# matter-labs/era-zkevm_test_harness

Measured on AMD Instinct MI355X. Metric: base-layer circuits/sec (2^20 rows); full-block synth wall-time 1/8 GPU, higher is better.
Workload: dtype u64 (Goldilocks, p = 2^64 - 2^32 + 1)

## Files before the change

### era_zkevm_test_harness_amd/csrc/poseidon2.cuh

```cuda
#pragma once
#include "gl64.cuh"
#include "../../include/zkw_poseidon2_params.h"

namespace p2 {
using gl::u32;
using gl::u64;

static __constant__ u64 c_rc[P2_TOTAL_ROUNDS * P2_WIDTH] = P2_ROUND_CONSTANTS_INIT;
static __constant__ u32 c_shift[P2_WIDTH] = P2_INTERNAL_DIAG_SHIFTS_INIT;

__host__ __device__ __forceinline__ u64 rc_at(int i) {
#if defined(__HIP_DEVICE_COMPILE__)
    return c_rc[i];
#else
    return P2_ROUND_CONSTANTS[i];
#endif
}
__host__ __device__ __forceinline__ u32 shift_at(int i) {
#if defined(__HIP_DEVICE_COMPILE__)
    return c_shift[i];
#else
    return P2_INTERNAL_DIAG_SHIFTS[i];
#endif
}

struct Wide {
    u64 lo;
    u32 hi;
};
GL_HD Wide wide(u64 x) { Wide r; r.lo = x; r.hi = 0; return r; }
GL_HD Wide wadd(Wide a, Wide b) {
    Wide r;
    r.lo = a.lo + b.lo;
    r.hi = a.hi + b.hi + (r.lo < a.lo ? 1u : 0u);
    return r;
}
GL_HD Wide wshl(Wide a, u32 s) {
    Wide r;
    r.lo = a.lo << s;
    r.hi = (a.hi << s) | (u32)(a.lo >> (64 - s));
    return r;
}
GL_HD u64 wreduce(Wide a) {
    u64 t = ((u64)a.hi << 32) - a.hi;
    u64 r = a.lo + t;
    u64 c = r < t ? gl::EPS : 0;
    return r + c;
}

GL_HD void m4w(const u64 x[4], Wide t[4]) {
    Wide t0 = wadd(wide(x[0]), wide(x[1])), t1 = wadd(wide(x[2]), wide(x[3]));
    Wide t2 = wadd(wshl(wide(x[1]), 1), t1), t3 = wadd(wshl(wide(x[3]), 1), t0);
    Wide t4 = wadd(wshl(t1, 2), t3), t5 = wadd(wshl(t0, 2), t2);
    t[0] = wadd(t3, t5); t[1] = t5; t[2] = wadd(t2, t4); t[3] = t4;
}

#if defined(__HIP_DEVICE_COMPILE__)
__device__ __forceinline__ u64 mad_acc(u32 a, u32 k, u64 acc) {
    u64 r, dead;
    asm("v_mad_u64_u32 %0, %1, %2, %3, %4" : "=v"(r), "=s"(dead) : "v"(a), "s"(k), "v"(acc));
    return r;
}
__device__ __forceinline__ u64 mad_acc1(u32 a, u64 acc) {
    u64 r, dead;
    asm("v_mad_u64_u32 %0, %1, %2, 1, %3" : "=v"(r), "=s"(dead) : "v"(a), "v"(acc));
    return r;
}
__device__ __forceinline__ u64 mad_acc2(u32 a, u64 acc) {
    u64 r, dead;
    asm("v_mad_u64_u32 %0, %1, %2, 2, %3" : "=v"(r), "=s"(dead) : "v"(a), "v"(acc));
    return r;
}
__device__ __forceinline__ u64 wp_reduce(u64 L, u64 H) {
    const u32 l0 = (u32)L, l1 = (u32)(L >> 32), h0 = (u32)H, h1 = (u32)(H >> 32);
    u32 n1, k, f;
    u64 c, c2, dead, r;
    asm("v_add_co_u32_e64 %0, %1, %2, %3" : "=v"(n1), "=s"(c) : "v"(l1), "v"(h0));
    asm("v_addc_co_u32_e64 %0, %1, %2, 0, %3" : "=v"(k), "=s"(dead) : "v"(h1), "s"(c));
    const u64 x = ((u64)n1 << 32) | l0;
    asm("v_mad_u64_u32 %0, %1, %2, -1, %3" : "=v"(r), "=s"(c2) : "v"(k), "v"(x));
    asm("v_cndmask_b32_e64 %0, 0, 1, %1" : "=v"(f) : "s"(c2));
    asm("v_mad_u64_u32 %0, %1, %2, -1, %3" : "=v"(r), "=s"(dead) : "v"(f), "v"(r));
    return r;
}
__device__ __forceinline__ void m4_plane(u32 a0, u32 a1, u32 a2, u32 a3, u64 y[4]) {
    const u64 t0 = mad_acc1(a0, (u64)a1), t1 = mad_acc1(a2, (u64)a3);
    const u64 t2 = mad_acc2(a1, t1), t3 = mad_acc2(a3, t0);
    const u64 t4 = (t1 << 2) + t3, t5 = (t0 << 2) + t2;
    y[0] = t3 + t5; y[1] = t5; y[2] = t2 + t4; y[3] = t4;
}
#endif

GL_HD void external(u64 s[12]) {
#if defined(__HIP_DEVICE_COMPILE__) && !defined(P2_LINEAR_WIDE)
    u64 L[12], H[12];
#pragma unroll
    for (int b = 0; b < 3; b++) {
        m4_plane((u32)s[4 * b], (u32)s[4 * b + 1], (u32)s[4 * b + 2], (u32)s[4 * b + 3], L + 4 * b);
        m4_plane((u32)(s[4 * b] >> 32), (u32)(s[4 * b + 1] >> 32), (u32)(s[4 * b + 2] >> 32), (u32)(s[4 * b + 3] >> 32), H + 4 * b);
    }
#pragma unroll
    for (int i = 0; i < 4; i++) {
        const u64 cl = L[i] + L[4 + i] + L[8 + i], ch = H[i] + H[4 + i] + H[8 + i];
#pragma unroll
        for (int b = 0; b < 3; b++) s[4 * b + i] = wp_reduce(L[4 * b + i] + cl, H[4 * b + i] + ch);
    }
#else
    Wide t[12];
    m4w(s, t); m4w(s + 4, t + 4); m4w(s + 8, t + 8);
#pragma unroll
    for (int i = 0; i < 4; i++) {
        Wide col = wadd(wadd(t[i], t[4 + i]), t[8 + i]);
        s[i] = wreduce(wadd(t[i], col)); s[4 + i] = wreduce(wadd(t[4 + i], col)); s[8 + i] = wreduce(wadd(t[8 + i], col));
    }
#endif
}

GL_HD void internal(u64 s[12]) {
    constexpr u32 SH[12] = P2_INTERNAL_DIAG_SHIFTS_INIT;
#if defined(__HIP_DEVICE_COMPILE__) && !defined(P2_LINEAR_WIDE)
    u64 sl = (u64)(u32)s[0], sh = s[0] >> 32;
#pragma unroll
    for (int i = 1; i < 12; i++) { sl = mad_acc1((u32)s[i], sl); sh = mad_acc1((u32)(s[i] >> 32), sh); }
#pragma unroll
    for (int i = 0; i < 12; i++) {
        const u64 l = SH[i] ? mad_acc((u32)s[i], 1u << SH[i], sl) : mad_acc1((u32)s[i], sl);
        const u64 h = SH[i] ? mad_acc((u32)(s[i] >> 32), 1u << SH[i], sh) : mad_acc1((u32)(s[i] >> 32), sh);
        s[i] = wp_reduce(l, h);
    }
#else
    Wide sum = wide(s[0]);
#pragma unroll
    for (int i = 1; i < 12; i++) sum = wadd(sum, wide(s[i]));
#pragma unroll
    for (int i = 0; i < 12; i++) s[i] = wreduce(wadd(SH[i] ? wshl(wide(s[i]), SH[i]) : wide(s[i]), sum));
#endif
}

#ifndef P2_SBOX_GROUP
#define P2_SBOX_GROUP 3
#endif
template <bool LAT = false>
GL_HD void full_round(u64 s[12], int r) {
#pragma unroll
    for (int i = 0; i < 12; i++) {
        s[i] = LAT ? gl::pow7_lat(gl::add_canon(s[i], rc_at(12 * r + i))) : gl::pow7(gl::add_canon(s[i], rc_at(12 * r + i)));
#if defined(__HIP_DEVICE_COMPILE__)
        if (!LAT && (i + 1) % P2_SBOX_GROUP == 0) __builtin_amdgcn_sched_barrier(0);
#endif
    }
    external(s);
}

template <bool LAT = false>
GL_HD void partial_round(u64 s[12], int r) {
    s[0] = LAT ? gl::pow7_lat(gl::add_canon(s[0], rc_at(12 * r))) : gl::pow7(gl::add_canon(s[0], rc_at(12 * r)));
    internal(s);
}

template <bool LAT = false>
GL_HD void permute(u64 s[12]) {
    external(s);
    int r = 0;
    for (int k = 0; k < P2_HALF_FULL_ROUNDS; k++, r++) full_round<LAT>(s, r);
    for (int k = 0; k < P2_PARTIAL_ROUNDS; k++, r++) partial_round<LAT>(s, r);
    for (int k = 0; k < P2_HALF_FULL_ROUNDS; k++, r++) full_round<LAT>(s, r);
}
GL_HD void permute_lat(u64 s[12]) { permute<true>(s); }

#if defined(__HIPCC__)
template <int CTRL>
__device__ __forceinline__ u32 dpp32(u32 v) {
    return (u32)__builtin_amdgcn_update_dpp((int)0, (int)v, CTRL, 0xF, 0xF, false);
}
template <int CTRL>
__device__ __forceinline__ u64 dpp64(u64 v) {
    u32 lo = dpp32<CTRL>((u32)v), hi = dpp32<CTRL>((u32)(v >> 32));
    return ((u64)hi << 32) | lo;
}
constexpr int QP_ROT1 = 1 | (2 << 2) | (3 << 4) | (0 << 6);
constexpr int QP_ROT2 = 2 | (3 << 2) | (0 << 4) | (1 << 6);
constexpr int QP_ROT3 = 3 | (0 << 2) | (1 << 4) | (2 << 6);
constexpr int QP_SWAP1 = 1 | (0 << 2) | (3 << 4) | (2 << 6);
constexpr int QP_BCAST0 = 0;
constexpr int ROW_ROR4 = 0x124, ROW_ROR8 = 0x128, ROW_ROR12 = 0x12C;

template <int CTRL>
__device__ __forceinline__ Wide wdpp(Wide a) {
    Wide r;
    r.lo = dpp64<CTRL>(a.lo);
    r.hi = dpp32<CTRL>(a.hi);
    return r;
}
__device__ __forceinline__ u64 add_rc_sched(u64 x, u64 c) {
    u32 r0, r1, m;
    asm("v_add_co_u32 %0, vcc, %3, %5\n\t"
        "v_addc_co_u32 %1, vcc, %4, %6, vcc\n\t"
        "v_cndmask_b32 %2, 0, -1, vcc\n\t"
        "v_add_co_u32 %0, vcc, %0, %2\n\t"
        "v_addc_co_u32 %1, vcc, 0, %1, vcc"
        : "=&v"(r0), "=&v"(r1), "=&v"(m)
        : "v"((u32)x), "v"((u32)(x >> 32)), "v"((u32)c), "v"((u32)(c >> 32))
        : "vcc");
    return ((u64)r1 << 32) | r0;
}
#if defined(GL_CHAIN_MUL_COMPILER_FORM)
#define P2_ROW_MUL gl::mul_sched
#else
#define P2_ROW_MUL gl::mul_vcc
#endif
__device__ __forceinline__ u64 pow7_sched(u64 x) {
    const u64 x2 = P2_ROW_MUL(x, x), x3 = P2_ROW_MUL(x2, x), x4 = P2_ROW_MUL(x2, x2);
    return P2_ROW_MUL(x3, x4);
}

struct Coop {
    u64 rc_full[2 * P2_HALF_FULL_ROUNDS];
    u32 ka, kb, kd;
    u32 shift;
    u32 rsh, hi_mask;
    bool active;
    bool first;
    bool second;

    __device__ __forceinline__ void init(int g) {
        active = g < 12;
        first = g == 0;
        second = g == 1;
#pragma unroll
        for (int k = 0; k < 2 * P2_HALF_FULL_ROUNDS; k++) {
            int round = k < P2_HALF_FULL_ROUNDS ? k : k + P2_PARTIAL_ROUNDS;
            rc_full[k] = active ? c_rc[12 * round + g] : 0;
        }
        bool even = (g & 1) == 0;
        ka = even ? 5u : 6u;
        kb = even ? 7u : 1u;
        kd = even ? 3u : 4u;
        shift = active ? c_shift[g] : 0;
        rsh = (32u - shift) & 31u;
        hi_mask = shift ? 0xffffffffu : 0u;
    }

    __device__ __forceinline__ u64 external(u64 x) const {
        u64 a = x, b = dpp64<QP_ROT1>(x), c = dpp64<QP_ROT2>(x), d = dpp64<QP_ROT3>(x);
        u64 L = (a & gl::EPS) * ka + (b & gl::EPS) * kb + (c & gl::EPS) + (d & gl::EPS) * kd;
        u64 H = (a >> 32) * ka + (b >> 32) * kb + (c >> 32) + (d >> 32) * kd;
        u32 r0, r1, t0, t1, t2, u0, u1, u2, e0, e1, e2;
        asm volatile(
            "v_add_co_u32 %3, vcc, %11, %13\n\t"
            "v_addc_co_u32 %4, vcc, 0, %14, vcc\n\t"
            "s_nop 0\n\t"
            "v_add_co_u32_dpp %5, vcc, %12, %12 row_ror:8 row_mask:0xf bank_mask:0xf\n\t"
            "v_addc_co_u32_dpp %6, vcc, %3, %3, vcc row_ror:8 row_mask:0xf bank_mask:0xf\n\t"
            "v_addc_co_u32_dpp %7, vcc, %4, %4, vcc row_ror:8 row_mask:0xf bank_mask:0xf\n\t"
            "v_add_co_u32_dpp %5, vcc, %5, %5 row_ror:4 row_mask:0xf bank_mask:0xf\n\t"
            "v_addc_co_u32_dpp %6, vcc, %6, %6, vcc row_ror:4 row_mask:0xf bank_mask:0xf\n\t"
            "v_addc_co_u32_dpp %7, vcc, %7, %7, vcc row_ror:4 row_mask:0xf bank_mask:0xf\n\t"
            "v_add_co_u32 %0, vcc, %12, %5\n\t"
            "v_addc_co_u32 %1, vcc, %3, %6, vcc\n\t"
            "v_addc_co_u32 %2, vcc, %4, %7, vcc\n\t"
            "v_sub_co_u32 %8, vcc, 0, %2\n\t"
            "v_subbrev_co_u32 %9, vcc, 0, %2, vcc\n\t"
            "v_add_co_u32 %0, vcc, %0, %8\n\t"
            "v_addc_co_u32 %1, vcc, %1, %9, vcc\n\t"
            "v_cndmask_b32 %10, 0, -1, vcc\n\t"
            "v_add_co_u32 %0, vcc, %0, %10\n\t"
            "v_addc_co_u32 %1, vcc, 0, %1, vcc"
            : "=&v"(r0), "=&v"(r1), "=&v"(t0), "=&v"(t1), "=&v"(t2), "=&v"(u0), "=&v"(u1), "=&v"(u2), "=&v"(e0), "=&v"(e1), "=&v"(e2)
            : "v"((u32)(L >> 32)), "v"((u32)L), "v"((u32)H), "v"((u32)(H >> 32))
            : "vcc");
        const u64 y = ((u64)r1 << 32) | r0;
        return active ? y : 0;
    }

    __device__ __forceinline__ u64 internal(u64 x) const {
        const u32 x0 = (u32)x, x1 = (u32)(x >> 32);
        u32 s0, s1, s2;
        const u32 zero = 0;
        asm volatile(
            "s_nop 1\n\t"
            "v_add_co_u32_dpp %0, vcc, %3, %3 row_ror:8 row_mask:0xf bank_mask:0xf\n\t"
            "v_addc_co_u32_dpp %1, vcc, %4, %4, vcc row_ror:8 row_mask:0xf bank_mask:0xf\n\t"
            "v_addc_co_u32 %2, vcc, 0, %5, vcc\n\t"
            "v_add_co_u32_dpp %0, vcc, %0, %0 row_ror:4 row_mask:0xf bank_mask:0xf\n\t"
            "v_addc_co_u32_dpp %1, vcc, %1, %1, vcc row_ror:4 row_mask:0xf bank_mask:0xf\n\t"
            "v_addc_co_u32_dpp %2, vcc, %2, %2, vcc row_ror:4 row_mask:0xf bank_mask:0xf\n\t"
            "v_add_co_u32_dpp %0, vcc, %0, %0 quad_perm:[2,3,0,1] row_mask:0xf bank_mask:0xf\n\t"
            "v_addc_co_u32_dpp %1, vcc, %1, %1, vcc quad_perm:[2,3,0,1] row_mask:0xf bank_mask:0xf\n\t"
            "v_addc_co_u32_dpp %2, vcc, %2, %2, vcc quad_perm:[2,3,0,1] row_mask:0xf bank_mask:0xf\n\t"
            "v_add_co_u32_dpp %0, vcc, %0, %0 quad_perm:[1,0,3,2] row_mask:0xf bank_mask:0xf\n\t"
            "v_addc_co_u32_dpp %1, vcc, %1, %1, vcc quad_perm:[1,0,3,2] row_mask:0xf bank_mask:0xf\n\t"
            "v_addc_co_u32_dpp %2, vcc, %2, %2, vcc quad_perm:[1,0,3,2] row_mask:0xf bank_mask:0xf"
            : "=&v"(s0), "=&v"(s1), "=&v"(s2)
            : "v"(x0), "v"(x1), "v"(zero)
            : "vcc");
        const u64 mlo = x << shift;
        const u32 m2 = (x1 >> rsh) & hi_mask;
        u32 r0, r1;
        u32 t0, t1, t2, t3;
        asm volatile(
            "v_add_co_u32 %0, vcc, %6, %9\n\t"
            "v_addc_co_u32 %1, vcc, %7, %10, vcc\n\t"
            "v_addc_co_u32 %2, vcc, %8, %11, vcc\n\t"
            "v_sub_co_u32 %3, vcc, 0, %2\n\t"
            "v_subbrev_co_u32 %4, vcc, 0, %2, vcc\n\t"
            "v_add_co_u32 %0, vcc, %0, %3\n\t"
            "v_addc_co_u32 %1, vcc, %1, %4, vcc\n\t"
            "v_cndmask_b32 %5, 0, -1, vcc\n\t"
            "v_add_co_u32 %0, vcc, %0, %5\n\t"
            "v_addc_co_u32 %1, vcc, 0, %1, vcc"
            : "=&v"(r0), "=&v"(r1), "=&v"(t0), "=&v"(t1), "=&v"(t2), "=&v"(t3)
            : "v"((u32)mlo), "v"((u32)(mlo >> 32)), "v"(m2), "v"(s0), "v"(s1), "v"(s2)
            : "vcc");
        const u64 y = ((u64)r1 << 32) | r0;
        return active ? y : 0;
    }

    __device__ __forceinline__ u64 permute(u64 x) const {
        x = external(x);
#pragma unroll
        for (int k = 0; k < P2_HALF_FULL_ROUNDS; k++) x = external(pow7_sched(add_rc_sched(x, rc_full[k])));
        for (int k = 0; k < P2_PARTIAL_ROUNDS; k++) {
            u64 rc = c_rc[12 * (P2_HALF_FULL_ROUNDS + k)];
            u64 sx = pow7_pair(add_rc_sched(x, rc));
            x = internal(first ? sx : x);
        }
#pragma unroll
        for (int k = 0; k < P2_HALF_FULL_ROUNDS; k++)
            x = external(pow7_sched(add_rc_sched(x, rc_full[P2_HALF_FULL_ROUNDS + k])));
        return x;
    }

    __device__ __forceinline__ u64 pow7_pair(u64 t) const {
        const u64 t0 = dpp64<QP_BCAST0>(t);
        const u64 x2 = P2_ROW_MUL(t0, t0);
        const u64 b = second ? x2 : t0;
        const u64 y = P2_ROW_MUL(x2, b);
        return P2_ROW_MUL(y, dpp64<QP_SWAP1>(y));
    }
};

template <class Put>
__device__ __forceinline__ u64 coop_flattened(const Coop& co, u64 x, u32 g, Put&& put) {
    if (co.active) put(g, gl::canon(x));
    x = co.external(x);
#pragma unroll
    for (int k = 0; k < P2_HALF_FULL_ROUNDS; k++) {
        x = co.external(pow7_sched(add_rc_sched(x, co.rc_full[k])));
        if (co.active) put(12 * (k + 1) + g, gl::canon(x));
    }
    for (int k = 0; k < P2_PARTIAL_ROUNDS; k++) {
        const u64 rc = c_rc[12 * (P2_HALF_FULL_ROUNDS + k)];
        const u64 sx = co.pow7_pair(add_rc_sched(x, rc));
        if (co.first) put(12 * (P2_HALF_FULL_ROUNDS + 1) + k, gl::canon(sx));
        x = co.internal(co.first ? sx : x);
    }
#pragma unroll
    for (int k = 0; k < P2_HALF_FULL_ROUNDS; k++) {
        x = co.external(pow7_sched(add_rc_sched(x, co.rc_full[P2_HALF_FULL_ROUNDS + k])));
        if (co.active) put(12 * (P2_HALF_FULL_ROUNDS + 1) + P2_PARTIAL_ROUNDS + 12 * k + g, gl::canon(x));
    }
    return gl::canon(x);
}


__device__ __forceinline__ u64 q4_mul(u64 a, u64 b) {
#if defined(GL_CHAIN_MUL_COMPILER_FORM)
    return gl::mul_lat(a, b);
#else
    return gl::mul_vcc(a, b);
#endif
}
__device__ __forceinline__ u64 q4_pow7(u64 x) {
    const u64 x2 = q4_mul(x, x), x3 = q4_mul(x2, x), x4 = q4_mul(x2, x2);
    return q4_mul(x3, x4);
}
template <int CTRL>
__device__ __forceinline__ u32 qdpp32(u32 v) {
    return (u32)__builtin_amdgcn_update_dpp((int)0, (int)v, CTRL, 0xF, 0xF, true);
}
template <int CTRL>
__device__ __forceinline__ u64 qdpp64(u64 v) {
    return ((u64)qdpp32<CTRL>((u32)(v >> 32)) << 32) | qdpp32<CTRL>((u32)v);
}

struct Coop4 {
    u64 rc_full[2 * P2_HALF_FULL_ROUNDS][3];
    u32 ka, kb, kd;
    u32 pw[3];
    bool first;
    bool second;

    __device__ __forceinline__ void init(int j) {
        first = j == 0;
        second = j == 1;
#pragma unroll
        for (int k = 0; k < 2 * P2_HALF_FULL_ROUNDS; k++) {
            int round = k < P2_HALF_FULL_ROUNDS ? k : k + P2_PARTIAL_ROUNDS;
#pragma unroll
            for (int c = 0; c < 3; c++) rc_full[k][c] = c_rc[12 * round + 4 * c + j];
        }
        bool even = (j & 1) == 0;
        ka = even ? 5u : 6u;
        kb = even ? 7u : 1u;
        kd = even ? 3u : 4u;
#pragma unroll
        for (int c = 0; c < 3; c++) pw[c] = 1u << c_shift[4 * c + j];
    }

#if defined(__HIP_DEVICE_COMPILE__)
    static __device__ __forceinline__ u64 mad_v(u32 a, u32 k, u64 acc) {
        u64 r, dead;
        asm("v_mad_u64_u32 %0, %1, %2, %3, %4" : "=v"(r), "=s"(dead) : "v"(a), "v"(k), "v"(acc));
        return r;
    }
    template <bool SC = false>
    static __device__ __forceinline__ u64 add_rc(u64 x, u32 c0, u32 c1);
#endif

    __device__ __forceinline__ u64 m4_plane(u32 a) const {
        const u32 b = qdpp32<QP_ROT1>(a), c = qdpp32<QP_ROT2>(a), d = qdpp32<QP_ROT3>(a);
#if defined(__HIP_DEVICE_COMPILE__)
        return mad_v(d, kd, mad_v(b, kb, mad_v(a, ka, (u64)c)));
#else
        return (u64)a * ka + (u64)b * kb + c + (u64)d * kd;
#endif
    }

    __device__ __forceinline__ void external(u64 x[3]) const {
#if defined(__HIP_DEVICE_COMPILE__)
        u64 L[3], H[3];
#pragma unroll
        for (int c = 0; c < 3; c++) { L[c] = m4_plane((u32)x[c]); H[c] = m4_plane((u32)(x[c] >> 32)); }
        const u64 cl = L[0] + L[1] + L[2], ch = H[0] + H[1] + H[2];
#pragma unroll
        for (int c = 0; c < 3; c++) x[c] = wp_reduce(L[c] + cl, H[c] + ch);
#endif
    }

    __device__ __forceinline__ void internal(u64 x[3]) const {
#if defined(__HIP_DEVICE_COMPILE__)
        const u64 pl = mad_acc1((u32)x[0], mad_acc1((u32)x[1], (u64)(u32)x[2]));
        const u64 ph = mad_acc1((u32)(x[0] >> 32), mad_acc1((u32)(x[1] >> 32), x[2] >> 32));
        u32 l0, l1, h0, h1;
        asm volatile(
            "s_nop 1\n\t"
            "v_add_co_u32_dpp %0, vcc, %4, %4 quad_perm:[2,3,0,1] row_mask:0xf bank_mask:0xf\n\t"
            "v_addc_co_u32_dpp %1, vcc, %5, %5, vcc quad_perm:[2,3,0,1] row_mask:0xf bank_mask:0xf\n\t"
            "v_add_co_u32_dpp %2, vcc, %6, %6 quad_perm:[2,3,0,1] row_mask:0xf bank_mask:0xf\n\t"
            "v_addc_co_u32_dpp %3, vcc, %7, %7, vcc quad_perm:[2,3,0,1] row_mask:0xf bank_mask:0xf\n\t"
            "v_add_co_u32_dpp %0, vcc, %0, %0 quad_perm:[1,0,3,2] row_mask:0xf bank_mask:0xf\n\t"
            "v_addc_co_u32_dpp %1, vcc, %1, %1, vcc quad_perm:[1,0,3,2] row_mask:0xf bank_mask:0xf\n\t"
            "v_add_co_u32_dpp %2, vcc, %2, %2 quad_perm:[1,0,3,2] row_mask:0xf bank_mask:0xf\n\t"
            "v_addc_co_u32_dpp %3, vcc, %3, %3, vcc quad_perm:[1,0,3,2] row_mask:0xf bank_mask:0xf"
            : "=&v"(l0), "=&v"(l1), "=&v"(h0), "=&v"(h1)
            : "v"((u32)pl), "v"((u32)(pl >> 32)), "v"((u32)ph), "v"((u32)(ph >> 32))
            : "vcc");
        const u64 sl = ((u64)l1 << 32) | l0, sh = ((u64)h1 << 32) | h0;
#pragma unroll
        for (int c = 0; c < 3; c++) x[c] = wp_reduce(mad_v((u32)x[c], pw[c], sl), mad_v((u32)(x[c] >> 32), pw[c], sh));
// ... 132 lines not shown
```

### era_zkevm_test_harness_amd/csrc/ram_circuit_kernels.cuh

```cuda
#pragma once
#include "../../include/zkw_ram_circuit_spec.h"
#include "../../include/zkw_decommit_sorter_circuit_spec.h"
#include "../../include/zkw_events_sorter_circuit_spec.h"
#include "ram_kernels.cuh"
#include "public_input_kernels.cuh"
#include "closed_form_kernels.cuh"

namespace zkw {

struct SynthJob {
    const zkw_ram_instance* inst;
    const zkw_mem_query* sorted_q;
    const zkw_mem_query* unsorted_q;
    const u64* unsorted_caps;
    const u64* sorted_caps;
    const u64* u_mark;
    const u64* s_mark;
    const u64* challenges;
    const u64* lhs_z;
    const u64* rhs_z;
    u64 n_block;
    u64* trace;
    u32* hist;
    u32* nd_tiles;
    const u64* public_input;
    const zkw_ram_instance* first_inst;
    u32 tail_clean;
};

constexpr int ROW_SLOTS[RC_NUM_ROW_TYPES] = RC_ROW_NUM_SLOTS_INIT;
constexpr int ROW_LOOKUPS[RC_NUM_ROW_TYPES] = RC_ROW_NUM_LOOKUPS_INIT;
static_assert(ROW_SLOTS[RC_ROW_PU] == 133 && ROW_SLOTS[RC_ROW_PS] == 130, "Poseidon2 rows: 130 gate variables (+3 spare in PU)");
static_assert(ROW_LOOKUPS[RC_ROW_PU] == 12 && ROW_LOOKUPS[RC_ROW_PS] == 12 && ROW_LOOKUPS[RC_ROW_A] == 12 &&
              ROW_LOOKUPS[RC_ROW_B] == 12 && ROW_LOOKUPS[RC_ROW_C] == 8 && ROW_LOOKUPS[RC_ROW_D] == 0,
              "lookup cells per cycle (56) are hard-wired in the fill kernels");
constexpr int LOOKUPS_PER_CYCLE = 56;

__device__ __forceinline__ u64 inv_or_zero(u64 x) { return gl::canon(x) ? gl::inv(x) : 0; }

struct RegsIn {
    const u64* uh;
    const u64* sh;
    u32 len;
};
__device__ __forceinline__ RegsIn regs_in(const zkw_ram_instance* in) {
    RegsIn r;
    const bool start = in->start_flag != 0;
    r.uh = start ? in->unsorted_queue_initial_state.head : in->hidden_fsm_input.current_unsorted_queue_state.head;
    r.sh = start ? in->sorted_queue_initial_state.head : in->hidden_fsm_input.current_sorted_queue_state.head;
    r.len = start ? in->unsorted_queue_initial_state.length : in->hidden_fsm_input.current_unsorted_queue_state.length;
    return r;
}

#define TR(col, row) trace[(size_t)(col) * n_rows + (row)]

__device__ __forceinline__ void zero_gap_row(u64* trace, size_t n_rows, size_t row) {
    for (int col = 0; col < RC_G + RC_L; col++) TR(col, row) = 0;
}
__device__ __forceinline__ void zero_gap_row_n(u64* trace, size_t n_rows, size_t row, int n_cols) {
    for (int col = 0; col < n_cols; col++) TR(col, row) = 0;
}

__device__ __forceinline__ void hist_bytes(u32* sh_hist, u32 x) {
    atomicAdd(&sh_hist[x & 0xFF], 1u);
    atomicAdd(&sh_hist[(x >> 8) & 0xFF], 1u);
    atomicAdd(&sh_hist[(x >> 16) & 0xFF], 1u);
    atomicAdd(&sh_hist[x >> 24], 1u);
}
__device__ __forceinline__ void put_bytes(u64* trace, size_t n_rows, size_t row, int col0, u32 x) {
    TR(col0, row) = x & 0xFF;
    TR(col0 + 1, row) = (x >> 8) & 0xFF;
    TR(col0 + 2, row) = (x >> 16) & 0xFF;
    TR(col0 + 3, row) = x >> 24;
}
__device__ __forceinline__ void hist_flush(u32* sh_hist, u32* g_hist) {
    __syncthreads();
    for (int t = threadIdx.x; t < 256; t += blockDim.x)
        if (sh_hist[t]) atomicAdd(&g_hist[t], sh_hist[t]);
}

__device__ __forceinline__ void fill_flattened_poseidon(u64* trace, size_t n_rows, size_t row, u64 s[12]) {
    int pos = 0;
#pragma unroll
    for (int k = 0; k < 12; k++) TR(pos++, row) = gl::canon(s[k]);
    p2::external(s);
    int r = 0;
    for (int k = 0; k < P2_HALF_FULL_ROUNDS; k++, r++) {
        p2::full_round(s, r);
#pragma unroll
        for (int j = 0; j < 12; j++) TR(pos + j, row) = gl::canon(s[j]);
        pos += 12;
    }
    for (int k = 0; k < P2_PARTIAL_ROUNDS; k++, r++) {
        s[0] = gl::pow7(gl::add_canon(s[0], p2::rc_at(12 * r)));
        TR(pos++, row) = gl::canon(s[0]);
        p2::internal(s);
    }
    for (int k = 0; k < P2_HALF_FULL_ROUNDS; k++, r++) {
        p2::full_round(s, r);
#pragma unroll
        for (int j = 0; j < 12; j++) TR(pos + j, row) = gl::canon(s[j]);
        pos += 12;
    }
}

template <int SIDE>
static __device__ __forceinline__ void k_ram_fill_poseidon(const VB& vb, const SynthJob* __restrict__ jobs, u32 capacity,
                                                          size_t n_rows) {
    __shared__ u32 sh_hist[256];
    for (int t = threadIdx.x; t < 256; t += blockDim.x) sh_hist[t] = 0;
    __syncthreads();
    const SynthJob job = jobs[vb.y];
    const u32 i = vb.x * blockDim.x + threadIdx.x;
    if (i < capacity) {
        u64* trace = job.trace;
        const zkw_ram_instance* in = job.inst;
        const size_t first = in->first_item, m = in->num_items;
        const bool can_pop = i < m;
        const size_t row = (size_t)(SIDE == 0 ? RC_ROW_PU : RC_ROW_PS) * RC_REGION_STRIDE(capacity) + i;
        const zkw_mem_query* qs = SIDE == 0 ? job.unsorted_q : job.sorted_q;
        const u64* caps = SIDE == 0 ? job.unsorted_caps : job.sorted_caps;
        u64 s[12];
        if (can_pop) {
            encode_raw_query(load_raw_query(qs + first + i), s);
        } else {
#pragma unroll
            for (int k = 0; k < 8; k++) s[k] = 0;
        }
        const RegsIn ri = regs_in(in);
        const u64* prev_cap = i == 0 ? (SIDE == 0 ? ri.uh : ri.sh) + 8 : caps + 4 * (first + (i - 1 < m ? i - 1 : m - 1));
#pragma unroll
        for (int k = 0; k < 4; k++) s[8 + k] = prev_cap[k];
        fill_flattened_poseidon(trace, n_rows, row, s);
        zkw_mem_query q;
        memset(&q, 0, sizeof q);
        if (can_pop) q = job.sorted_q[first + i];
        if (SIDE == 0) {
            TR(RC_PU_idx, row) = q.index; TR(RC_PU_v0, row) = q.value[0]; TR(RC_PU_v1, row) = q.value[1];
            put_bytes(trace, n_rows, row, RC_PU_idx_b0, q.index);
            put_bytes(trace, n_rows, row, RC_PU_v0_b0, q.value[0]);
            put_bytes(trace, n_rows, row, RC_PU_v1_b0, q.value[1]);
            hist_bytes(sh_hist, q.index); hist_bytes(sh_hist, q.value[0]); hist_bytes(sh_hist, q.value[1]);
        } else {
            if (!job.tail_clean) for (int c = 130; c < RC_G; c++) TR(c, row) = 0;
            put_bytes(trace, n_rows, row, RC_PS_ts_b0, q.timestamp);
            put_bytes(trace, n_rows, row, RC_PS_page_b0, q.page);
            put_bytes(trace, n_rows, row, RC_PS_v4_b0, q.value[4]);
            hist_bytes(sh_hist, q.timestamp); hist_bytes(sh_hist, q.page); hist_bytes(sh_hist, q.value[4]);
        }
        if (!job.tail_clean) for (int c = RC_G + 12; c < RC_G + RC_L; c++) TR(c, row) = 0;
    } else if (i < RC_REGION_STRIDE(capacity)) {
        if (!job.tail_clean) zero_gap_row(job.trace, n_rows, (size_t)(SIDE == 0 ? RC_ROW_PU : RC_ROW_PS) * RC_REGION_STRIDE(capacity) + i);
    }
    hist_flush(sh_hist, job.hist);
}

struct CycleCtx {
    bool can_pop;
    zkw_mem_query q, pq;
    u64 eu[8], es[8];
    u64 p_val[5];
    u32 p_ptr;
};

__device__ __forceinline__ void load_query(const zkw_mem_query* src, zkw_mem_query& dst) {
    const uint4* s = reinterpret_cast<const uint4*>(src);
    uint4* d = reinterpret_cast<uint4*>(&dst);
    d[0] = s[0]; d[1] = s[1]; d[2] = s[2];
}

__device__ __forceinline__ void cycle_ctx(const SynthJob& job, u32 i, CycleCtx& c, bool want_eu) {
    const zkw_ram_instance* in = job.inst;
    const size_t first = in->first_item, m = in->num_items;
    c.can_pop = i < m;
    memset(&c.q, 0, sizeof c.q);
    memset(&c.pq, 0, sizeof c.pq);
#pragma unroll
    for (int k = 0; k < 8; k++) { c.eu[k] = 0; c.es[k] = 0; }
    if (c.can_pop) {
        load_query(job.sorted_q + first + i, c.q);
        encode_mem_query(c.q, c.es);
        if (want_eu) encode_raw_query(load_raw_query(job.unsorted_q + first + i), c.eu);
    }
    if (i == 0) {
        const zkw_ram_fsm& f = in->hidden_fsm_input;
        c.pq.timestamp = f.previous_sorting_key[0]; c.pq.index = f.previous_sorting_key[1]; c.pq.page = f.previous_sorting_key[2];
        for (int k = 0; k < 8; k++) c.pq.value[k] = f.previous_value[k];
        c.pq.value_is_pointer = f.previous_is_ptr ? 1 : 0;
    } else if (i - 1 < m) {
        load_query(job.sorted_q + first + i - 1, c.pq);
    }
    u64 pe[8];
    encode_mem_query(c.pq, pe);
#pragma unroll
    for (int k = 0; k < 5; k++) c.p_val[k] = pe[3 + k];
    c.p_ptr = c.pq.value_is_pointer ? 1 : 0;
}

__device__ __forceinline__ u64 acc_before(const u64* z, size_t first, size_t m, u32 i, u64 fsm_in) {
    return i == 0 ? fsm_in : z[first + (i - 1 < m ? i - 1 : m - 1)];
}

static __device__ __forceinline__ void k_ram_fill_A(const VB& vb, const SynthJob* __restrict__ jobs, u32 capacity, size_t n_rows) {
    __shared__ u32 sh_hist[256];
    sh_hist[threadIdx.x] = 0;
    __syncthreads();
    const SynthJob job = jobs[vb.y];
    const u32 i = vb.x * blockDim.x + threadIdx.x;
    const u64* lhs_z_all = job.lhs_z;
    const u64* rhs_z_all = job.rhs_z;
    const size_t n_total = job.n_block;
    if (i < capacity) {
        u64* trace = job.trace;
        const zkw_ram_instance* in = job.inst;
        const size_t first = in->first_item, m = in->num_items, row = (size_t)RC_ROW_A * RC_REGION_STRIDE(capacity) + i;
        CycleCtx c;
        cycle_ctx(job, i, c, true);
        const u64 rw = c.q.rw_flag ? 1 : 0, ptr = c.q.value_is_pointer ? 1 : 0;
#pragma unroll
        for (int k = 0; k < 8; k++) { TR(RC_A_eu0 + k, row) = c.eu[k]; TR(RC_A_ts + k, row) = c.es[k]; }
        for (int r = 0; r < 2; r++) {
            const u64* ch = job.challenges + 9 * r;
            u64 lc = ch[8], rc = ch[8];
#pragma unroll
            for (int k = 0; k < 8; k++) {
                lc = gl::add(lc, gl::mul(c.eu[k], ch[k]));
                rc = gl::add(rc, gl::mul(c.es[k], ch[k]));
            }
            const u64 pl = acc_before(lhs_z_all + (size_t)r * n_total, first, m, i, in->hidden_fsm_input.lhs_accumulator[r]);
            const u64 pr = acc_before(rhs_z_all + (size_t)r * n_total, first, m, i, in->hidden_fsm_input.rhs_accumulator[r]);
            const u64 nl = gl::canon(gl::mul(pl, lc)), nr = gl::canon(gl::mul(pr, rc));
            const int o = r * (RC_A_lc1 - RC_A_lc0);
#pragma unroll
            for (int k = 1; k < 9; k++) TR(RC_A_G_c0_1 + (k - 1) + r * (RC_A_G_c1_1 - RC_A_G_c0_1), row) = ch[k];
            TR(RC_A_lc0 + o, row) = gl::canon(lc); TR(RC_A_P_lhs0 + o, row) = pl; TR(RC_A_nl0 + o, row) = nl;
            TR(RC_A_lhs0 + o, row) = c.can_pop ? nl : pl;
            TR(RC_A_rc0 + o, row) = gl::canon(rc); TR(RC_A_P_rhs0 + o, row) = pr; TR(RC_A_nr0 + o, row) = nr;
            TR(RC_A_rhs0 + o, row) = c.can_pop ? nr : pr;
        }
        TR(RC_A_rw, row) = rw; TR(RC_A_ptr, row) = ptr; TR(RC_A_idx, row) = c.q.index;
        TR(RC_A_v2, row) = c.q.value[2]; TR(RC_A_v3, row) = c.q.value[3]; TR(RC_A_v0, row) = c.q.value[0];
        TR(RC_A_v5_b3c, row) = c.q.value[5] >> 24; TR(RC_A_can_pop, row) = c.can_pop ? 1 : 0;
        put_bytes(trace, n_rows, row, RC_A_v2_b0, c.q.value[2]);
        put_bytes(trace, n_rows, row, RC_A_v3_b0, c.q.value[3]);
        put_bytes(trace, n_rows, row, RC_A_v5_b0, c.q.value[5]);
        hist_bytes(sh_hist, c.q.value[2]); hist_bytes(sh_hist, c.q.value[3]); hist_bytes(sh_hist, c.q.value[5]);
        constexpr int NA = ROW_SLOTS[RC_ROW_A];
        if (!job.tail_clean) {
            for (int col = NA; col < RC_G; col++) TR(col, row) = 0;
            for (int col = RC_G + 12; col < RC_G + RC_L; col++) TR(col, row) = 0;
        }
    } else if (i < RC_REGION_STRIDE(capacity)) {
        if (!job.tail_clean) zero_gap_row(job.trace, n_rows, (size_t)RC_ROW_A * RC_REGION_STRIDE(capacity) + i);
    }
    hist_flush(sh_hist, job.hist);
}

static __device__ __forceinline__ void k_ram_fill_B(const VB& vb, const SynthJob* __restrict__ jobs, u32 capacity, size_t n_rows) {
    __shared__ u32 sh_hist[256];
    sh_hist[threadIdx.x] = 0;
    __syncthreads();
    const SynthJob job = jobs[vb.y];
    const u32 i = vb.x * blockDim.x + threadIdx.x;
    if (i < capacity) {
        u64* trace = job.trace;
        const size_t row = (size_t)RC_ROW_B * RC_REGION_STRIDE(capacity) + i;
        CycleCtx c;
        cycle_ctx(job, i, c, false);
        put_bytes(trace, n_rows, row, RC_B_v6_b0, c.q.value[6]);
        put_bytes(trace, n_rows, row, RC_B_v7_b0, c.q.value[7]);
        TR(RC_B_es4, row) = c.es[4]; TR(RC_B_v1, row) = c.q.value[1]; TR(RC_B_v5_b3c, row) = c.q.value[5] >> 24;
        TR(RC_B_es5, row) = c.es[5]; TR(RC_B_v2, row) = c.q.value[2];
        TR(RC_B_es6, row) = c.es[6]; TR(RC_B_v3, row) = c.q.value[3];
        const u32 d0 = c.q.timestamp - c.pq.timestamp;
        TR(RC_B_d0, row) = d0; put_bytes(trace, n_rows, row, RC_B_d0_b0, d0);
        TR(RC_B_bw0, row) = c.q.timestamp < c.pq.timestamp ? 1 : 0;
        TR(RC_B_ts, row) = c.q.timestamp; TR(RC_B_P_ts, row) = c.pq.timestamp;
        hist_bytes(sh_hist, c.q.value[6]); hist_bytes(sh_hist, c.q.value[7]); hist_bytes(sh_hist, d0);
        constexpr int NB = ROW_SLOTS[RC_ROW_B];
        if (!job.tail_clean) {
            for (int col = NB; col < RC_G; col++) TR(col, row) = 0;
            for (int col = RC_G + 12; col < RC_G + RC_L; col++) TR(col, row) = 0;
        }
    } else if (i < RC_REGION_STRIDE(capacity)) {
        if (!job.tail_clean) zero_gap_row(job.trace, n_rows, (size_t)RC_ROW_B * RC_REGION_STRIDE(capacity) + i);
    }
    hist_flush(sh_hist, job.hist);
}

__device__ __forceinline__ bool nd_flag(bool can_pop, const zkw_mem_query& q) {
    return can_pop && q.timestamp == 0 && q.page == RC_HEAP_PAGE && q.rw_flag && !q.value_is_pointer;
}

static __device__ __forceinline__ void k_ram_nd_tiles(const VB& vb, const SynthJob* __restrict__ jobs, u32 capacity) {
    __shared__ u32 sh[4];
    const SynthJob job = jobs[vb.y];
    const u32 i = vb.x * blockDim.x + threadIdx.x;
    const zkw_ram_instance* in = job.inst;
    bool f = false;
    if (i < capacity && i < in->num_items) {
        zkw_mem_query q;
        load_query(job.sorted_q + in->first_item + i, q);
        f = nd_flag(true, q);
    }
    u32 cnt = __popcll(__ballot(f));
    if ((threadIdx.x & 63) == 0) sh[threadIdx.x >> 6] = cnt;
    __syncthreads();
    if (threadIdx.x == 0) job.nd_tiles[vb.x] = sh[0] + sh[1] + sh[2] + sh[3];
}
static __device__ __forceinline__ void k_ram_nd_scan(const VB& vb, const SynthJob* __restrict__ jobs, int n_jobs, u32 n_tiles) {
    u32* t = jobs[vb.x].nd_tiles;
    const int lane = threadIdx.x;
    u32 acc = 0;
    for (u32 base = 0; base < n_tiles; base += 64) {
        const u32 k = base + lane;
        const u32 v = k < n_tiles ? t[k] : 0;
        u32 incl = v;
        for (int off = 1; off < 64; off <<= 1) {
            const u32 up = __shfl_up(incl, off);
            if (lane >= off) incl += up;
        }
        if (k < n_tiles) t[k] = acc + incl - v;
        acc += __shfl(incl, 63);
    }
}

static __device__ __forceinline__ void k_ram_fill_C(const VB& vb, const SynthJob* __restrict__ jobs, u32 capacity, size_t n_rows) {
    __shared__ u32 sh_hist[256];
    __shared__ u32 sh_wave[4];
    sh_hist[threadIdx.x] = 0;
    __syncthreads();
    const SynthJob job = jobs[vb.y];
    const u32 i = vb.x * blockDim.x + threadIdx.x;
    const bool live = i < capacity;
    CycleCtx c;
    c.can_pop = false;
    bool nd = false;
    if (live) {
        cycle_ctx(job, i, c, false);
        nd = nd_flag(c.can_pop, c.q);
    }
    const unsigned long long bal = __ballot(nd);
    const int lane = threadIdx.x & 63, wave = threadIdx.x >> 6;
    if (lane == 0) sh_wave[wave] = __popcll(bal);
    __syncthreads();
    u32 before = __popcll(bal & ((1ull << lane) - 1));
    for (int w = 0; w < wave; w++) before += sh_wave[w];
    if (live) {
        u64* trace = job.trace;
        const zkw_ram_instance* in = job.inst;
        const size_t row = (size_t)RC_ROW_C * RC_REGION_STRIDE(capacity) + i;
        const u64 rw = c.q.rw_flag ? 1 : 0, ptr = c.q.value_is_pointer ? 1 : 0;
        const u64 bw0 = c.q.timestamp < c.pq.timestamp ? 1 : 0;
        const u64 t1 = (u64)c.pq.index + bw0, bw1 = (u64)c.q.index < t1 ? 1 : 0;
        const u32 d1 = (u32)((u64)c.q.index - t1);
        const u64 t2 = (u64)c.pq.page + bw1, bw2 = (u64)c.q.page < t2 ? 1 : 0;
        const u32 d2 = (u32)((u64)c.q.page - t2);
        TR(RC_C_d1, row) = d1; put_bytes(trace, n_rows, row, RC_C_d1_b0, d1);
        TR(RC_C_d2, row) = d2; put_bytes(trace, n_rows, row, RC_C_d2_b0, d2);
        hist_bytes(sh_hist, d1); hist_bytes(sh_hist, d2);
        TR(RC_C_bw1, row) = bw1; TR(RC_C_bw2, row) = bw2; TR(RC_C_bw0, row) = bw0;
        TR(RC_C_idx, row) = c.q.index; TR(RC_C_P_idx, row) = c.pq.index;
        TR(RC_C_page, row) = c.q.page; TR(RC_C_P_page, row) = c.pq.page;
        TR(RC_C_can_pop, row) = c.can_pop ? 1 : 0;
        u64 x[14];
        x[0] = gl::canon(gl::sub(c.q.index, c.pq.index));
        x[1] = gl::canon(gl::sub(c.q.page, c.pq.page));
        const u64 val[5] = {c.es[3], c.es[4], c.es[5], c.es[6], c.es[7]};
#pragma unroll
        for (int k = 0; k < 5; k++) { x[2 + k] = gl::canon(gl::sub(val[k], c.p_val[k])); x[7 + k] = val[k]; }
        x[12] = c.q.timestamp;
        x[13] = gl::canon(gl::sub(c.q.page, RC_HEAP_PAGE));
        u64 pre[14], acc = 1;
#pragma unroll
        for (int k = 0; k < 14; k++) { pre[k] = acc; acc = gl::mul(acc, x[k] ? x[k] : 1); }
        u64 inv = gl::inv(acc), w[14];
#pragma unroll
        for (int k = 13; k >= 0; k--) {
            w[k] = x[k] ? gl::canon(gl::mul(inv, pre[k])) : 0;
            inv = gl::mul(inv, x[k] ? x[k] : 1);
        }
        const u64 z_idx = x[0] == 0, z_page = x[1] == 0, same = z_idx & z_page;
        TR(RC_C_w_idx, row) = w[0]; TR(RC_C_z_idx, row) = z_idx;
        TR(RC_C_w_page, row) = w[1]; TR(RC_C_z_page, row) = z_page; TR(RC_C_same, row) = same;
        const int C_VAL[5] = {RC_C_es3, RC_C_es4, RC_C_es5, RC_C_es6, RC_C_v4};
        const int C_PVAL[5] = {RC_C_P_es3, RC_C_P_es4, RC_C_P_es5, RC_C_P_es6, RC_C_P_v4};
        const int C_WEQ[5] = {RC_C_w_eq0, RC_C_w_eq1, RC_C_w_eq2, RC_C_w_eq3, RC_C_w_eq4};
        const int C_ZEQ[5] = {RC_C_z_eq0, RC_C_z_eq1, RC_C_z_eq2, RC_C_z_eq3, RC_C_z_eq4};
        const int C_WZ[5] = {RC_C_w_z0, RC_C_w_z1, RC_C_w_z2, RC_C_w_z3, RC_C_w_z4};
        const int C_ZZ[5] = {RC_C_z_z0, RC_C_z_z1, RC_C_z_z2, RC_C_z_z3, RC_C_z_z4};
        u64 zeq[5], zz[5];
#pragma unroll
        for (int k = 0; k < 5; k++) {
            zeq[k] = x[2 + k] == 0; zz[k] = x[7 + k] == 0;
            TR(C_VAL[k], row) = val[k]; TR(C_PVAL[k], row) = c.p_val[k];
            TR(C_WEQ[k], row) = w[2 + k]; TR(C_ZEQ[k], row) = zeq[k];
            TR(C_WZ[k], row) = w[7 + k]; TR(C_ZZ[k], row) = zz[k];
        }
        const u64 peq = ptr == c.p_ptr, eq_a = zeq[0] & zeq[1] & zeq[2], value_equal = eq_a & zeq[3] & zeq[4] & peq;
        const u64 zz_a = zz[0] & zz[1] & zz[2], all_zero = zz_a & zz[3] & zz[4] & (1 - ptr);
        TR(RC_C_ptr, row) = ptr; TR(RC_C_P_ptr, row) = c.p_ptr; TR(RC_C_peq, row) = peq;
        TR(RC_C_eq_a, row) = eq_a; TR(RC_C_value_equal, row) = value_equal;
        TR(RC_C_zz_a, row) = zz_a; TR(RC_C_all_zero, row) = all_zero; TR(RC_C_rw, row) = rw;
        TR(RC_C_ts, row) = c.q.timestamp; TR(RC_C_w_ts, row) = w[12]; TR(RC_C_z_ts, row) = x[12] == 0;
        TR(RC_C_w_heap, row) = w[13]; TR(RC_C_z_heap, row) = x[13] == 0; TR(RC_C_nd, row) = nd ? 1 : 0;
        const u64 p_cnt = (u64)in->hidden_fsm_input.num_nondeterministic_writes + job.nd_tiles[vb.x] + before;
        TR(RC_C_P_cnt, row) = p_cnt; TR(RC_C_cnt, row) = p_cnt + (nd ? 1 : 0);
        constexpr int NC = ROW_SLOTS[RC_ROW_C];
        if (!job.tail_clean) {
            for (int col = NC; col < RC_G; col++) TR(col, row) = 0;
            for (int col = RC_G + 8; col < RC_G + RC_L; col++) TR(col, row) = 0;
        }
    } else if (i < RC_REGION_STRIDE(capacity)) {
        if (!job.tail_clean) zero_gap_row(job.trace, n_rows, (size_t)RC_ROW_C * RC_REGION_STRIDE(capacity) + i);
    }
    if (vb.x == 0 && threadIdx.x == 0)
        for (int l = 5; l < 8; l++) { hist_bytes(sh_hist, job.inst->hidden_fsm_input.previous_value[l]); hist_bytes(sh_hist, job.inst->hidden_fsm_output.previous_value[l]); }
    hist_flush(sh_hist, job.hist);
}

__device__ __forceinline__ void ram_boundary_block(const SynthJob& job, u32 capacity, size_t n_rows);
constexpr int RC_D_TILES = 4;
static __device__ __forceinline__ void k_ram_fill_D(const VB& vb, const SynthJob* __restrict__ jobs, u32 n_jobs, u32 n_tiles, u32 capacity, size_t n_rows) {
    if (vb.x < n_jobs) {
        __builtin_amdgcn_s_setprio(3);
        ram_boundary_block(jobs[vb.x], capacity, n_rows);
        return;
    }
    const SynthJob& job = jobs[(vb.x - n_jobs) / n_tiles];
    const u32 i0 = ((vb.x - n_jobs) % n_tiles) * (RC_D_TILES * 256) + threadIdx.x;
    const size_t rs = RC_REGION_STRIDE(capacity);
    u64* trace = job.trace;
    const zkw_ram_instance* in = job.inst;
    const size_t m = in->num_items;
    const RegsIn ri = regs_in(in);
    u64 len[RC_D_TILES], pre[RC_D_TILES], w[RC_D_TILES];
    u64 acc = 1;
#pragma unroll
    for (int k = 0; k < RC_D_TILES; k++) {
        const u32 i = i0 + 256 * k;
        len[k] = (u64)ri.len - (i < m ? i : m);
        pre[k] = acc;
        acc = gl::mul(acc, len[k] ? len[k] : 1);
    }
    acc = gl::inv(acc);
#pragma unroll
    for (int k = RC_D_TILES - 1; k >= 0; k--) {
        w[k] = len[k] ? gl::canon(gl::mul(acc, pre[k])) : 0;
        acc = gl::mul(acc, len[k] ? len[k] : 1);
    }
#pragma unroll
    for (int k = 0; k < RC_D_TILES; k++) {
        const u32 i = i0 + 256 * k;
        if (i >= capacity) {
            if (i < rs && !job.tail_clean) zero_gap_row(job.trace, n_rows, (size_t)RC_ROW_D * rs + i);
            continue;
        }
        const size_t row = (size_t)RC_ROW_D * rs + i;
        const size_t rPU = (size_t)RC_ROW_PU * rs + i, rPS = (size_t)RC_ROW_PS * rs + i;
        const bool can_pop = i < m;
        const u64 p_len = len[k];
        const u64 w_len = w[k], z_len = p_len == 0;
        TR(RC_D_P_len_u, row) = p_len; TR(RC_D_w_lu, row) = w_len; TR(RC_D_z_lu, row) = z_len;
        TR(RC_D_P_len_s, row) = p_len; TR(RC_D_w_ls, row) = w_len; TR(RC_D_z_ls, row) = z_len;
        TR(RC_D_can_pop, row) = can_pop ? 1 : 0;
        TR(RC_D_len_u, row) = p_len - (can_pop ? 1 : 0); TR(RC_D_len_s, row) = p_len - (can_pop ? 1 : 0);
        const size_t p = i - 1 < m ? i - 1 : m - 1, rPUp = (size_t)RC_ROW_PU * rs + p, rPSp = (size_t)RC_ROW_PS * rs + p;
#pragma unroll
        for (int e = 0; e < 12; e++) {
            const u64 uo = TR(RC_PU_uo0 + e, rPU);
            const u64 so = TR(RC_PS_so0 + e, rPS);
            const u64 a = i == 0 ? ri.uh[e] : TR(RC_PU_uo0 + e, rPUp), b = i == 0 ? ri.sh[e] : TR(RC_PS_so0 + e, rPSp);
            const int o = 3 * e;
            TR(RC_D_uo0 + o, row) = uo; TR(RC_D_P_uh0 + o, row) = a; TR(RC_D_uh0 + o, row) = can_pop ? uo : a;
            TR(RC_D_so0 + o, row) = so; TR(RC_D_P_sh0 + o, row) = b; TR(RC_D_sh0 + o, row) = can_pop ? so : b;
        }
        constexpr int ND = ROW_SLOTS[RC_ROW_D];
        if (!job.tail_clean) for (int col = ND; col < RC_G + RC_L; col++) TR(col, row) = 0;
    }
}

constexpr int TAIL_CHUNKS = 8;
constexpr int RC_BOUNDARY_ROWS = RC_NUM_ROW_TYPES - RC_ROWS_PER_CYCLE;
constexpr int RC_CF_LOOKUP_CELLS = 24;
static_assert(RC_BOUNDARY_ROWS % 2 == 0, "the tail's 16-byte stores start below the boundary rows");
static __device__ __forceinline__ void k_ram_fill_tail(const VB& vb, const SynthJob* __restrict__ jobs, u32 capacity, size_t n_rows) {
    constexpr u32 PER_JOB = (RC_G + RC_L + 1) * TAIL_CHUNKS;
    const u32 bid = vb.x % PER_JOB;
    const SynthJob& job = jobs[vb.x / PER_JOB];
    u64* trace = job.trace;
    const int col = bid / TAIL_CHUNKS, ch = bid % TAIL_CHUNKS;
    if (col < RC_G + RC_L) {
        if (job.tail_clean) return;
        const size_t bnd = (size_t)RC_BOUNDARY_ROW(capacity) + RC_BOUNDARY_ROWS;
        const size_t n_pairs = (n_rows - bnd) / 2;
        const size_t per = (n_pairs + TAIL_CHUNKS - 1) / TAIL_CHUNKS, lo = ch * per, hi = lo + per < n_pairs ? lo + per : n_pairs;
        ulonglong2* c2 = reinterpret_cast<ulonglong2*>(trace + (size_t)col * n_rows + bnd);
        const ulonglong2 z = make_ulonglong2(0, 0);
        for (size_t k = lo + threadIdx.x; k < hi; k += 256) c2[k] = z;
        return;
    }
    u64* m = trace + (size_t)RC_MULT_COL * n_rows;
    const size_t per = (n_rows + TAIL_CHUNKS - 1) / TAIL_CHUNKS, lo = ch * per, hi = lo + per < n_rows ? lo + per : n_rows;
    for (size_t r = lo + threadIdx.x; r < (job.tail_clean && hi > 256 ? (lo < 256 ? 256 : lo) : hi); r += 256) {
        u64 v = 0;
        if (r < 256) {
            v = job.hist[r];
            if (r == 0) v += (u64)RC_L * n_rows - (u64)LOOKUPS_PER_CYCLE * capacity - RC_CF_LOOKUP_CELLS;
        }
        m[r] = v;
    }
}

static __constant__ rc_link c_links[RC_NUM_LINKS] = RC_LINKS_INIT;
static __constant__ uint8_t c_is_poseidon[RC_NUM_ROW_TYPES] = RC_ROW_IS_POSEIDON_INIT;
ZKW_CF_TABLES(RC, rc)

__device__ __forceinline__ void ram_fill_register_rows(const SynthJob& job, u32 capacity, size_t n_rows) {
    const u64* lhs_z_all = job.lhs_z;
    const u64* rhs_z_all = job.rhs_z;
    const size_t n_total = job.n_block;
    u64* trace = job.trace;
    const zkw_ram_instance* in = job.inst;
    const zkw_ram_fsm& fi = in->hidden_fsm_input;
    const size_t first = in->first_item, m = in->num_items;
    const size_t bin = (size_t)RC_BOUNDARY_ROW(capacity) + RC_ROWOFF_BND_IN, bout = bin - RC_ROWOFF_BND_IN + RC_ROWOFF_BND_OUT;
    const RegsIn ri = regs_in(in);
    for (int k = 0; k < 12; k++) { TR(RC_BND_IN_uh0 + k, bin) = ri.uh[k]; TR(RC_BND_IN_sh0 + k, bin) = ri.sh[k]; }
    TR(RC_BND_IN_len_u, bin) = ri.len; TR(RC_BND_IN_len_s, bin) = ri.len;
    for (int r = 0; r < 2; r++) { TR(RC_BND_IN_lhs0 + r, bin) = fi.lhs_accumulator[r]; TR(RC_BND_IN_rhs0 + r, bin) = fi.rhs_accumulator[r]; }
    zkw_mem_query pq;
    memset(&pq, 0, sizeof pq);
    for (int k = 0; k < 8; k++) pq.value[k] = fi.previous_value[k];
    u64 pe[8];
    encode_mem_query(pq, pe);
    TR(RC_BND_IN_ts, bin) = fi.previous_sorting_key[0]; TR(RC_BND_IN_idx, bin) = fi.previous_sorting_key[1];
    TR(RC_BND_IN_page, bin) = fi.previous_sorting_key[2];
    TR(RC_BND_IN_es3, bin) = pe[3]; TR(RC_BND_IN_es4, bin) = pe[4]; TR(RC_BND_IN_es5, bin) = pe[5];
    TR(RC_BND_IN_es6, bin) = pe[6]; TR(RC_BND_IN_v4, bin) = pe[7];
    TR(RC_BND_IN_ptr, bin) = fi.previous_is_ptr ? 1 : 0; TR(RC_BND_IN_cnt, bin) = fi.num_nondeterministic_writes;
    for (int r = 0; r < 2; r++)
        for (int k = 1; k < 9; k++) TR(RC_BND_IN_G_c0_1 + 8 * r + (k - 1), bin) = job.challenges[9 * r + k];
    const size_t last = first + m - 1;
    const bool padded = m < capacity;
    const u64 len_out = (u64)ri.len - m;
    for (int k = 0; k < 12; k++) {
        TR(RC_BND_OUT_uh0 + k, bout) = job.u_mark[k];
        TR(RC_BND_OUT_sh0 + k, bout) = job.s_mark[k];
        TR(RC_BND_OUT_tail_u0 + k, bout) = in->unsorted_queue_initial_state.tail[k];
        TR(RC_BND_OUT_tail_s0 + k, bout) = in->sorted_queue_initial_state.tail[k];
    }
    TR(RC_BND_OUT_len_u, bout) = len_out; TR(RC_BND_OUT_len_s, bout) = len_out;
    for (int r = 0; r < 2; r++) {
        TR(RC_BND_OUT_lhs0 + r, bout) = lhs_z_all[(size_t)r * n_total + last];
        TR(RC_BND_OUT_rhs0 + r, bout) = rhs_z_all[(size_t)r * n_total + last];
    }
    zkw_mem_query lq;
    memset(&lq, 0, sizeof lq);
    if (!padded) lq = job.sorted_q[last];
    u64 le[8];
    encode_mem_query(lq, le);
    TR(RC_BND_OUT_ts, bout) = lq.timestamp; TR(RC_BND_OUT_idx, bout) = lq.index; TR(RC_BND_OUT_page, bout) = lq.page;
    TR(RC_BND_OUT_es3, bout) = le[3]; TR(RC_BND_OUT_es4, bout) = le[4]; TR(RC_BND_OUT_es5, bout) = le[5];
    TR(RC_BND_OUT_es6, bout) = le[6]; TR(RC_BND_OUT_v4, bout) = le[7];
    TR(RC_BND_OUT_ptr, bout) = lq.value_is_pointer ? 1 : 0;
    TR(RC_BND_OUT_cnt, bout) = TR(RC_C_cnt, (size_t)RC_ROW_C * RC_REGION_STRIDE(capacity) + capacity - 1);
    TR(RC_BND_OUT_completion, bout) = in->completion_flag ? 1 : 0;
    TR(RC_BND_OUT_w_end, bout) = inv_or_zero(len_out); TR(RC_BND_OUT_z_end, bout) = len_out == 0;
}

__device__ __forceinline__ void ram_value_row(u64* trace, size_t n_rows, size_t row, int v0, int b0, int e3) {
    zkw_mem_query q;
    memset(&q, 0, sizeof q);
    for (int k = 0; k < 8; k++) q.value[k] = (u32)TR(v0 + k, row);
    for (int l = 5; l < 8; l++)
        for (int k = 0; k < 4; k++) {
            const u64 b = (q.value[l] >> (8 * k)) & 0xFF;
            TR(b0 + 4 * (l - 5) + k, row) = b;
        }
    if (e3 < 0) return;
    u64 e[8];
    encode_mem_query(q, e);
    for (int k = 0; k < 4; k++) TR(e3 + k, row) = e[3 + k];
}

__device__ __forceinline__ void ram_boundary_block(const SynthJob& job, u32 capacity, size_t n_rows) {
    {
        u64* trace = job.trace;
        const size_t bnd = (size_t)RC_BOUNDARY_ROW(capacity);
        for (int k = threadIdx.x; k < (RC_G + RC_L) * RC_BOUNDARY_ROWS; k += CF_THREADS) TR(k / RC_BOUNDARY_ROWS, bnd + k % RC_BOUNDARY_ROWS) = 0;
    }
    __syncthreads();
    __shared__ u64 sh_oi[RAM_INPUT_ENC_LEN], sh_fi[RAM_FSM_ENC_LEN], sh_fo[RAM_FSM_ENC_LEN], sh_flags[2];
    if (threadIdx.x == 0) ram_fill_register_rows(job, capacity, n_rows);
    if (threadIdx.x == 64) {
        int m = put_queue12(job.first_inst->unsorted_queue_initial_state, sh_oi);
        m += put_queue12(job.first_inst->sorted_queue_initial_state, sh_oi + m);
        sh_oi[m] = job.first_inst->non_deterministic_bootloader_memory_snapshot_length;
    }
    if (threadIdx.x == 128) ram_encode_fsm(job.inst->hidden_fsm_input, sh_fi);
    if (threadIdx.x == 192) {
        ram_encode_fsm(job.inst->hidden_fsm_output, sh_fo);
        sh_flags[0] = job.inst->start_flag ? 1 : 0;
        sh_flags[1] = job.inst->completion_flag ? 1 : 0;
    }
    __syncthreads();
    const CfSpec S = ZKW_CF_SPEC(RC, rc, c_is_poseidon);
    const CfSources src = {sh_oi, sh_fi, sh_fo, sh_flags, nullptr};
    u64* trace = job.trace;
    cf_fill_block(S, trace, n_rows, (size_t)RC_BOUNDARY_ROW(capacity), src, [&](int rt, size_t row) {
        if (threadIdx.x != 0) return;
        if (rt == RC_ROW_VIN) ram_value_row(trace, n_rows, row, RC_VIN_VIN_v0, RC_VIN_VIN_v5_b0, RC_VIN_VIN_e3);
        if (rt == RC_ROW_VOUT) ram_value_row(trace, n_rows, row, RC_VOUT_VOUT_v0, RC_VOUT_VOUT_v5_b0, -1);
    });
}

static __constant__ rc_term c_terms[RC_NUM_TERMS] = RC_TERMS_INIT;
static __constant__ rc_constraint c_cons[RC_NUM_CONSTRAINTS] = RC_CONSTRAINTS_INIT;
static __constant__ uint16_t c_row_first[RC_NUM_ROW_TYPES + 1] = RC_ROW_FIRST_CONSTRAINT_INIT;
static __constant__ rc_term c_ds_terms[DS_NUM_TERMS] = DS_TERMS_INIT;
static __constant__ rc_constraint c_ds_cons[DS_NUM_CONSTRAINTS] = DS_CONSTRAINTS_INIT;
static __constant__ uint16_t c_ds_row_first[DS_NUM_ROW_TYPES + 1] = DS_ROW_FIRST_CONSTRAINT_INIT;
static __constant__ uint8_t c_ds_is_poseidon[DS_NUM_ROW_TYPES] = DS_ROW_IS_POSEIDON_INIT;
static __constant__ rc_link c_ds_links[DS_NUM_LINKS] = DS_LINKS_INIT;

struct SpecRam {
    static constexpr int G = RC_G, L = RC_L, ROWS_PER_CYCLE = RC_ROWS_PER_CYCLE, NUM_ROW_TYPES = RC_NUM_ROW_TYPES, NUM_LINKS = RC_NUM_LINKS;
    static constexpr int OFF_BIN = RC_ROWOFF_BND_IN, OFF_BOUT = RC_ROWOFF_BND_OUT;
    __device__ static const rc_term* terms() { return c_terms; }
    __device__ static const rc_constraint* cons() { return c_cons; }
    __device__ static const uint16_t* row_first() { return c_row_first; }
    __device__ static const uint8_t* is_poseidon() { return c_is_poseidon; }
    __device__ static const rc_link* links() { return c_links; }
};
ZKW_CF_TABLES(DS, ds)
struct SpecDecommitSorter {
    static constexpr int G = DS_G, L = DS_L, ROWS_PER_CYCLE = DS_ROWS_PER_CYCLE, NUM_ROW_TYPES = DS_NUM_ROW_TYPES, NUM_LINKS = DS_NUM_LINKS;
    static constexpr int OFF_BIN = DS_ROWOFF_BND_IN, OFF_BOUT = DS_ROWOFF_BND_OUT;
    __device__ static const rc_term* terms() { return c_ds_terms; }
    __device__ static const rc_constraint* cons() { return c_ds_cons; }
    __device__ static const uint16_t* row_first() { return c_ds_row_first; }
    __device__ static const uint8_t* is_poseidon() { return c_ds_is_poseidon; }
    __device__ static const rc_link* links() { return c_ds_links; }
    ZKW_CF_SPEC_MEMBERS(DS, ds)
};
static __constant__ rc_term c_es_terms[ES_NUM_TERMS] = ES_TERMS_INIT;
static __constant__ rc_constraint c_es_cons[ES_NUM_CONSTRAINTS] = ES_CONSTRAINTS_INIT;
static __constant__ uint16_t c_es_row_first[ES_NUM_ROW_TYPES + 1] = ES_ROW_FIRST_CONSTRAINT_INIT;
static __constant__ uint8_t c_es_is_poseidon[ES_NUM_ROW_TYPES] = ES_ROW_IS_POSEIDON_INIT;
static __constant__ rc_link c_es_links[ES_NUM_LINKS] = ES_LINKS_INIT;
ZKW_CF_TABLES(ES, es)
struct SpecEventsSorter {
    static constexpr int G = ES_G, L = ES_L, ROWS_PER_CYCLE = ES_ROWS_PER_CYCLE, NUM_ROW_TYPES = ES_NUM_ROW_TYPES, NUM_LINKS = ES_NUM_LINKS;
    static constexpr int OFF_BIN = ES_ROWOFF_BND_IN, OFF_BOUT = ES_ROWOFF_BND_OUT;
    __device__ static const rc_term* terms() { return c_es_terms; }
    __device__ static const rc_constraint* cons() { return c_es_cons; }
    __device__ static const uint16_t* row_first() { return c_es_row_first; }
    __device__ static const uint8_t* is_poseidon() { return c_es_is_poseidon; }
    __device__ static const rc_link* links() { return c_es_links; }
    ZKW_CF_SPEC_MEMBERS(ES, es)
};

struct CheckResult {
    unsigned long long violations;
    unsigned long long first_bad;
};

__device__ __forceinline__ void flag_bad(CheckResult* res, u64 kind, u64 idx, u64 row) {
    atomicAdd(&res->violations, 1ull);
    atomicMin(&res->first_bad, (kind << 56) | (idx << 32) | row);
}

constexpr int CHK_ROWS = 64;

template <class S>
__device__ __forceinline__ size_t spec_row(int rt, u32 capacity, u32 i) {
    const size_t rs = RC_REGION_STRIDE(capacity);
    return rt < S::ROWS_PER_CYCLE ? (size_t)rt * rs + i : (size_t)S::ROWS_PER_CYCLE * rs + (rt - S::ROWS_PER_CYCLE);
}

template <class S>
static __global__ __launch_bounds__(64) void k_check_rows(const u64* __restrict__ trace, u32 capacity, size_t n_rows, CheckResult* res) {
    extern __shared__ __attribute__((aligned(16))) u64 tile[];
    constexpr int CHK_COLS = S::G + S::L;
    const int rt = blockIdx.y;
    const bool per_cycle = rt < S::ROWS_PER_CYCLE;
    const u32 n_in_region = per_cycle ? capacity : 1;
    const u32 i = blockIdx.x * CHK_ROWS + threadIdx.x;
    if (blockIdx.x * CHK_ROWS >= n_in_region) return;
    const bool live = i < n_in_region;
    const size_t row = spec_row<S>(rt, capacity, per_cycle ? i : 0);
    for (int c = 0; c < CHK_COLS; c++) {
        u64 v = live ? TR(c, row) : 0;
        tile[c * CHK_ROWS + threadIdx.x] = v;
        if (live && (v >= gl::P || (c >= S::G && v > 255))) flag_bad(res, 3, c, row);
    }
    __syncthreads();
    if (!live) return;
#define CELLV(c) tile[(c) * CHK_ROWS + threadIdx.x]
    for (int k = S::row_first()[rt]; k < S::row_first()[rt + 1]; k++) {
        const rc_constraint cn = S::cons()[k];
        u64 acc = 0;
        for (int t = 0; t < cn.n_terms; t++) {
            const rc_term* tm = &S::terms()[cn.first_term + t];
            u64 v = tm->coef;
            for (int f = 0; f < tm->nf; f++) v = gl::mul(v, CELLV(tm->f[f]));
            acc = gl::add(acc, v);
        }
        if (gl::canon(acc) != 0) flag_bad(res, 1, k, row);
    }
    if (S::is_poseidon()[rt]) {
        u64 s[12];
#pragma unroll
        for (int k = 0; k < 12; k++) s[k] = CELLV(k);
        int pos = 12, r = 0;
        bool ok = true;
        p2::external(s);
        for (int k = 0; k < P2_HALF_FULL_ROUNDS; k++, r++) {
            p2::full_round(s, r);
#pragma unroll
            for (int j = 0; j < 12; j++) ok &= gl::canon(s[j]) == CELLV(pos + j);
            pos += 12;
        }
        for (int k = 0; k < P2_PARTIAL_ROUNDS; k++, r++) {
            s[0] = gl::pow7(gl::add_canon(s[0], p2::rc_at(12 * r)));
            ok &= gl::canon(s[0]) == CELLV(pos);
            pos++;
            p2::internal(s);
        }
        for (int k = 0; k < P2_HALF_FULL_ROUNDS; k++, r++) {
            p2::full_round(s, r);
#pragma unroll
            for (int j = 0; j < 12; j++) ok &= gl::canon(s[j]) == CELLV(pos + j);
            pos += 12;
        }
        if (!ok) flag_bad(res, 2, 0, row);
    }
#undef CELLV
}

template <class S>
static __global__ __launch_bounds__(256) void k_check_links(const u64* __restrict__ trace, u32 capacity, size_t n_rows, CheckResult* res) {
    const u32 i = blockIdx.x * blockDim.x + threadIdx.x;
    if (i >= capacity) return;
    const size_t rs = RC_REGION_STRIDE(capacity), bnd = (size_t)S::ROWS_PER_CYCLE * rs;
    for (int l = 0; l < S::NUM_LINKS; l++) {
        const rc_link k = S::links()[l];
        if (k.kind == 3) {
            if (i == capacity - 1 && TR(k.col_a, bnd + S::OFF_BOUT) != TR(k.col_b, (size_t)k.row_b * rs + i))
                flag_bad(res, 4, l, bnd + S::OFF_BOUT);
            continue;
        }
        if (k.kind == 4) {
            if (i == 0 && TR(k.col_a, spec_row<S>(k.row_a, capacity, 0)) != TR(k.col_b, bnd + S::OFF_BOUT))
                flag_bad(res, 4, l, spec_row<S>(k.row_a, capacity, 0));
            continue;
        }
        if (k.kind == 5) {
            if (i == 0 && TR(k.col_a, spec_row<S>(k.row_a, capacity, 0)) != TR(k.col_b, spec_row<S>(k.row_b, capacity, 0)))
                flag_bad(res, 4, l, spec_row<S>(k.row_a, capacity, 0));
            continue;
        }
        const size_t ra = (size_t)k.row_a * rs + i;
        const u64 a = TR(k.col_a, ra);
        u64 b;
        if (k.kind == 0) b = TR(k.col_b, (size_t)k.row_b * rs + i);
        else if (k.kind == 1) b = i ? TR(k.col_b, (size_t)k.row_b * rs + i - 1) : TR(k.bin_col, bnd + S::OFF_BIN);
        else b = TR(k.col_b, bnd + S::OFF_BIN);
        if (a != b) flag_bad(res, 4, l, ra);
    }
}

template <class S>
static __global__ __launch_bounds__(256) void k_check_lookups(const u64* __restrict__ trace, u32 capacity, size_t n_rows,
                                                       u32* __restrict__ hist, CheckResult* res) {
    __shared__ u32 sh_hist[256];
    sh_hist[threadIdx.x] = 0;
    __syncthreads();
    const size_t rs = RC_REGION_STRIDE(capacity), pad0 = (size_t)S::ROWS_PER_CYCLE * rs + (S::NUM_ROW_TYPES - S::ROWS_PER_CYCLE);
    const size_t stride = (size_t)gridDim.x * blockDim.x;
    for (size_t r = (size_t)blockIdx.x * blockDim.x + threadIdx.x; r < n_rows; r += stride) {
        for (int c = S::G; c < S::G + S::L; c++) {
            const u64 v = TR(c, r);
            if (v > 255) flag_bad(res, 3, c, r); else atomicAdd(&sh_hist[v], 1u);
        }
        if (r >= pad0 || (r < (size_t)S::ROWS_PER_CYCLE * rs && r % rs >= capacity))
            for (int c = 0; c < S::G; c++)
                if (TR(c, r) != 0) { flag_bad(res, 6, c, r); break; }
    }
    __syncthreads();
    if (sh_hist[threadIdx.x]) atomicAdd(&hist[threadIdx.x], sh_hist[threadIdx.x]);
}
static __global__ void k_check_mult(const u64* __restrict__ trace, size_t n_rows, int mult_col, const u32* __restrict__ hist, CheckResult* res) {
    const size_t stride = (size_t)gridDim.x * blockDim.x;
    for (size_t r = (size_t)blockIdx.x * blockDim.x + threadIdx.x; r < n_rows; r += stride) {
        const u64 want = r < 256 ? hist[r] : 0;
        if (TR(mult_col, r) != want) flag_bad(res, 5, 0, r);
    }
}

#undef TR
}
```

### era_zkevm_test_harness_amd/csrc/zkw_api.hip

```cpp
#include "zkw_ctx.h"
#include "circuit_check_host.h"
#include "closed_forms_host.h"
#include "callstack_kernels.cuh"
#include "vm_kernels.cuh"
#include "radix_sort.cuh"

static thread_local std::string g_last_error;

#undef fail
int zkw_fail(int code, const char* fmt, ...) {
    char buf[512];
    va_list ap;
    va_start(ap, fmt);
    vsnprintf(buf, sizeof buf, fmt, ap);
    va_end(ap);
    g_last_error = buf;
    return code;
}

#define fail zkw_fail

struct AllocCache {
    static constexpr size_t SMALL_MAX = size_t(256) << 20;
    static constexpr int MAX_DEV = 16;
// ... 1156 lines not shown
    for (size_t b = 0; b < n_blocks; b++) {
        const size_t lo = w->offsets[b], n = w->offsets[b + 1] - lo;
        const size_t last_inst = w->inst_offsets[b + 1] - 1;
        fs[b] = FsJob{w->unsorted_marks + 12 * last_inst, w->sorted_marks + 12 * last_inst, (u32)n, (u32)n,
                      w->challenges + 18 * b};
    }
    ZKW_TRY(dev_fs(ctx, fs, 12, 9));
    w->z_valid = false;
    for (size_t b0 = 0; b0 < n_blocks;) {
        size_t b1 = b0 + 1;
        while (b1 < n_blocks && w->offsets[b1 + 1] - w->offsets[b0] <= w->zcap) b1++;
        ZKW_TRY(ram_gp_blocks(ctx, w, b0, b1, w->zbuf_l, w->zbuf_r));
        const size_t base = w->offsets[b0];
        std::vector<RamBlock> blocks(b1 - b0);
        size_t max_inst = 0;
        for (size_t b = b0; b < b1; b++) {
            const size_t lo = w->offsets[b], n = w->offsets[b + 1] - lo;
            const size_t n_inst = w->inst_offsets[b + 1] - w->inst_offsets[b];
            if (n_inst > max_inst) max_inst = n_inst;
            blocks[b - b0] = RamBlock{w->unsorted_q,
                                      w->perm + lo,
                                      w->unsorted_marks + 12 * w->inst_offsets[b],
                                      w->sorted_marks + 12 * w->inst_offsets[b],
                                      w->zbuf_l + 2 * (lo - base),
                                      w->zbuf_r + 2 * (lo - base),
                                      w->instances + w->inst_offsets[b],
                                      w->nondet_counts + w->inst_offsets[b],
                                      n,
                                      w->capacity,
                                      n_nondet ? n_nondet[b] : 0u};
        }
        RamBlock* d_blocks = nullptr;
        ZKW_TRY(ctx->upload("ram_blocks", blocks, &d_blocks));
        const unsigned gx = (unsigned)(max_inst < 64 ? max_inst : 64), gy = (unsigned)(b1 - b0);
        { Prof _p(ctx, "k_ram_count_nondet"); ZKW_LAUNCH_2D(ctx, k_ram_count_nondet, gx, gy, 256, d_blocks); }
        ZKW_TRY(launch_check("k_ram_count_nondet"));
        { Prof _p(ctx, "k_ram_instances"); ZKW_LAUNCH_2D(ctx, k_ram_instances, blocks_for(max_inst, 64), gy, 64, d_blocks); }
        ZKW_TRY(launch_check("k_ram_instances"));
        b0 = b1;
    }
    const size_t ni = w->n_instances;
    { Prof _p(ctx, "k_ram_commitments"); ZKW_LAUNCH(ctx, k_ram_commitments, blocks_for(4 * ni, 64), 64, w->instances, ni, w->compact_forms); }
    ZKW_TRY(launch_check("k_ram_commitments"));
    { Prof _p(ctx, "k_commit_encodings"); ZKW_LAUNCH(ctx, k_commit_encodings, blocks_for(ni, 64), 64, w->compact_forms, ni, (u32)COMPACT_FORM_LEN, w->public_inputs); }
    return launch_check("k_commit_encodings");
}

extern "C" int zkw_ram_build_instances_batch(zkw_ctx* ctx, const zkw_mem_query* q, const uint64_t* block_offsets,
                                             size_t n_blocks, uint32_t capacity, const uint32_t* n_nondet,
                                             zkw_ram_witness** out) {
    if (!ctx || !q || !block_offsets || !out || n_blocks == 0 || capacity == 0)
        return fail(ZKW_ERR_INVALID, "zkw_ram_build_instances_batch: bad argument");
    HIP_TRY(hipSetDevice(ctx->device));
    const uint64_t base = block_offsets[0];
    std::vector<uint64_t> offs(n_blocks + 1), ioffs(n_blocks + 1, 0);
    for (size_t b = 0; b <= n_blocks; b++) offs[b] = block_offsets[b] - base;
    for (size_t b = 0; b < n_blocks; b++) {
        if (block_offsets[b + 1] <= block_offsets[b])
            return fail(ZKW_ERR_INVALID, "block %zu is empty: the VM must have made memory requests "
                                         "(W/ram_permutation.rs:43-46)", b);
        ioffs[b + 1] = ioffs[b] + (offs[b + 1] - offs[b] + capacity - 1) / capacity;
    }
    const size_t total = offs[n_blocks];
    if (total >= (1ull << 32)) return fail(ZKW_ERR_INVALID, "more than 2^32-1 queries in one batch");
    zkw_ram_witness* w = *out;
    if (w && (w->ctx != ctx || w->offsets != offs || w->capacity != capacity)) {
        zkw_ram_witness_free(w);
        w = nullptr;
        *out = nullptr;
    }
    if (!w) {
        w = new zkw_ram_witness();
        w->ctx = ctx;
        w->offsets = offs;
        w->inst_offsets = ioffs;
        w->capacity = capacity;
        w->total = total;
        w->n_instances = ioffs[n_blocks];
        int rc = ram_alloc(w, n_blocks);
        if (rc != ZKW_OK) {
            w->release();
            delete w;
            return rc;
        }
    }
    const zkw_mem_query* d_q = nullptr;
    int rc = ctx->in("ram_q", q + base, total, &d_q);
    if (rc == ZKW_OK) rc = ram_run(ctx, w, d_q, n_nondet);
    if (rc == ZKW_OK) rc = ctx->sync_if_host();
    if (rc != ZKW_OK) {
        if (!*out) {
            w->release();
            delete w;
        }
        return rc;
    }
    if (!*out) ctx_retain(ctx);
    *out = w;
    return ZKW_OK;
}

extern "C" int zkw_ram_build_instances(zkw_ctx* ctx, const zkw_mem_query* q, size_t n, uint32_t capacity,
                                       uint32_t num_non_deterministic_heap_queries, zkw_ram_witness** out) {
    uint64_t offsets[2] = {0, n};
    return zkw_ram_build_instances_batch(ctx, q, offsets, 1, capacity, &num_non_deterministic_heap_queries, out);
}

extern "C" size_t zkw_ram_witness_num_instances(const zkw_ram_witness* w) { return w ? w->n_instances : 0; }
extern "C" size_t zkw_ram_witness_num_items(const zkw_ram_witness* w) { return w ? w->total : 0; }

static int ram_sorted_queries(const zkw_ram_witness* cw) {
    zkw_ram_witness* w = const_cast<zkw_ram_witness*>(cw);
    if (w->sorted_valid) return ZKW_OK;
    zkw_ctx* ctx = w->ctx;
    HIP_TRY(hipSetDevice(ctx->device));
    const size_t t = w->total;
    if (!w->sorted_q && dev_malloc((void**)&w->sorted_q, (t + 1) * sizeof(zkw_mem_query)) != hipSuccess)
        return fail(ZKW_ERR_OOM, "no room for the sorted queries (%zu bytes): read ZKW_RAM_SORTED_QUERIES from a smaller batch", t * sizeof(zkw_mem_query));
    { Prof _p(ctx, "k_gather_encode"); ZKW_LAUNCH(ctx, k_gather_encode, blocks_for(t, 256), 256, w->unsorted_q, w->perm, t, w->sorted_q, (u64*)nullptr); }
    ZKW_TRY(launch_check("k_gather_encode"));
    w->sorted_valid = true;
    return ZKW_OK;
}

static int ram_full_chains(const zkw_ram_witness* cw) {
    zkw_ram_witness* w = const_cast<zkw_ram_witness*>(cw);
    if (w->z_valid) return ZKW_OK;
    zkw_ctx* ctx = w->ctx;
    HIP_TRY(hipSetDevice(ctx->device));
    const size_t t = w->total;
    if (!w->lhs_z) {
        if (dev_malloc((void**)&w->lhs_z, (t + 1) * 16) != hipSuccess || dev_malloc((void**)&w->rhs_z, (t + 1) * 16) != hipSuccess)
            return fail(ZKW_ERR_OOM, "no room for the grand-product chains (%zu bytes): read ZKW_RAM_*_Z from a smaller batch", 2 * t * 16);
    }
    ZKW_TRY(ram_gp_blocks(ctx, w, 0, w->offsets.size() - 1, w->lhs_z, w->rhs_z));
    w->z_valid = true;
    return ZKW_OK;
}

static int ram_encodings(const zkw_ram_witness* cw) {
    zkw_ram_witness* w = const_cast<zkw_ram_witness*>(cw);
    if (w->enc_valid) return ZKW_OK;
    zkw_ctx* ctx = w->ctx;
    HIP_TRY(hipSetDevice(ctx->device));
    const size_t t = w->total;
    if (!w->unsorted_enc) {
        if (dev_malloc((void**)&w->unsorted_enc, (t + 1) * 64) != hipSuccess || dev_malloc((void**)&w->sorted_enc, (t + 1) * 64) != hipSuccess)
            return fail(ZKW_ERR_OOM, "no room for the materialised encodings (%zu bytes): read ZKW_RAM_*_ENC from a smaller batch", 2 * t * 64);
    }
    ZKW_TRY(ram_sorted_queries(cw));
    ZKW_TRY(dev_encode(ctx, w->unsorted_q, t, w->unsorted_enc));
    ZKW_TRY(dev_encode(ctx, w->sorted_q, t, w->sorted_enc));
    w->enc_valid = true;
    return ZKW_OK;
}

static int ram_full_tails(const zkw_ram_witness* cw) {
    zkw_ram_witness* w = const_cast<zkw_ram_witness*>(cw);
    if (w->tails_valid) return ZKW_OK;
    ZKW_TRY(ram_encodings(cw));
    zkw_ctx* ctx = w->ctx;
    HIP_TRY(hipSetDevice(ctx->device));
    const size_t t = w->total;
    if (!w->unsorted_tails) {
        if (dev_malloc((void**)&w->unsorted_tails, (t + 1) * 96) != hipSuccess || dev_malloc((void**)&w->sorted_tails, (t + 1) * 96) != hipSuccess)
            return fail(ZKW_ERR_OOM, "no room for the expanded queue tails (%zu bytes): read ZKW_RAM_*_TAILS from a smaller batch", 2 * t * 96);
    }
    u64* d_off = nullptr;
    ZKW_TRY(ctx->upload("tails_off", w->offsets, &d_off));
    const int nq = (int)(w->offsets.size() - 1);
    { Prof _p(ctx, "k_tails_expand"); ZKW_LAUNCH(ctx, k_tails_expand, blocks_for(t, 64), 64, w->unsorted_enc, w->unsorted_caps, d_off, nq, t, w->unsorted_tails); }
    ZKW_TRY(launch_check("k_tails_expand"));
    { Prof _p(ctx, "k_tails_expand"); ZKW_LAUNCH(ctx, k_tails_expand, blocks_for(t, 64), 64, w->sorted_enc, w->sorted_caps, d_off, nq, t, w->sorted_tails); }
    ZKW_TRY(launch_check("k_tails_expand"));
    w->tails_valid = true;
    return ZKW_OK;
}

static const void* ram_array(const zkw_ram_witness* w, int what, size_t* bytes, bool materialize = true, int* rc = nullptr) {
    const size_t t = w->total, nb = w->offsets.size() - 1;
    int st = ZKW_OK;
    const void* p = nullptr;
#define RAM_LAZY(fn, field) do { if (materialize) { st = fn(w); if (st == ZKW_OK) p = w->field; } } while (0)
    switch (what) {
        case ZKW_RAM_SORTED_QUERIES: *bytes = t * sizeof(zkw_mem_query); RAM_LAZY(ram_sorted_queries, sorted_q); break;
        case ZKW_RAM_UNSORTED_ENC: *bytes = t * 64; RAM_LAZY(ram_encodings, unsorted_enc); break;
        case ZKW_RAM_SORTED_ENC: *bytes = t * 64; RAM_LAZY(ram_encodings, sorted_enc); break;
        case ZKW_RAM_UNSORTED_TAILS: *bytes = t * 96; RAM_LAZY(ram_full_tails, unsorted_tails); break;
        case ZKW_RAM_SORTED_TAILS: *bytes = t * 96; RAM_LAZY(ram_full_tails, sorted_tails); break;
        case ZKW_RAM_CHALLENGES: *bytes = nb * 18 * 8; p = w->challenges; break;
        case ZKW_RAM_LHS_Z: *bytes = t * 16; RAM_LAZY(ram_full_chains, lhs_z); break;
        case ZKW_RAM_RHS_Z: *bytes = t * 16; RAM_LAZY(ram_full_chains, rhs_z); break;
        case ZKW_RAM_INSTANCES: *bytes = w->n_instances * sizeof(zkw_ram_instance); p = w->instances; break;
        case ZKW_RAM_COMPACT_FORMS: *bytes = w->n_instances * COMPACT_FORM_LEN * 8; p = w->compact_forms; break;
        case ZKW_RAM_PUBLIC_INPUTS: *bytes = w->n_instances * 32; p = w->public_inputs; break;
        default: *bytes = 0; st = ZKW_ERR_INVALID; break;
    }
#undef RAM_LAZY
    if (rc) *rc = st;
    return p;
}

extern "C" size_t zkw_ram_witness_bytes(const zkw_ram_witness* w, int what) {
    size_t b = 0;
    if (w) (void)ram_array(w, what, &b, false);
    return b;
}

extern "C" const void* zkw_ram_witness_device_ptr(const zkw_ram_witness* w, int what) {
    size_t b = 0;
    return w ? ram_array(w, what, &b) : nullptr;
}

extern "C" int zkw_ram_witness_get(const zkw_ram_witness* w, int what, void* dst, size_t dst_bytes) {
    if (!w || !dst) return fail(ZKW_ERR_INVALID, "zkw_ram_witness_get: null argument");
    size_t bytes = 0;
    int st = ZKW_OK;
    const void* src = ram_array(w, what, &bytes, true, &st);
    if (st == ZKW_ERR_INVALID) return fail(ZKW_ERR_INVALID, "zkw_ram_witness_get: unknown array %d", what);
    if (st != ZKW_OK) return st;
    if (!src) return fail(ZKW_ERR_INVALID, "zkw_ram_witness_get: array %d is empty", what);
    if (dst_bytes < bytes) return fail(ZKW_ERR_INVALID, "zkw_ram_witness_get: need %zu bytes, got %zu", bytes, dst_bytes);
    zkw_ctx* ctx = w->ctx;
    HIP_TRY(hipSetDevice(ctx->device));
    HIP_TRY(ctx->copy_async(dst, src, bytes, ctx->ptr_mode == ZKW_PTR_DEVICE ? hipMemcpyDeviceToDevice : hipMemcpyDeviceToHost));
    return ctx->sync_if_host();
}

extern "C" void zkw_ram_witness_free(zkw_ram_witness* w) {
    if (!w) return;
    (void)hipSetDevice(w->ctx->device);
    (void)hipStreamSynchronize(w->ctx->stream);
    w->release();
    zkw_ctx* owner = w->ctx;
    delete w;
    ctx_release(owner);
}


extern "C" int zkw_trace_create_with_columns(zkw_ctx* ctx, size_t n_rows, size_t n_cols, size_t n_slots, zkw_trace** out) {
    if (!ctx || !out || n_rows < 256 || n_slots == 0 || n_cols == 0 || n_cols > 4096)
        return fail(ZKW_ERR_INVALID, "zkw_trace_create: bad argument");
    HIP_TRY(hipSetDevice(ctx->device));
    zkw_trace* t = new zkw_trace();
    t->ctx = ctx;
    t->n_rows = n_rows;
    t->n_cols = n_cols;
    t->n_slots = n_slots;
    t->slot_tag.reset(new std::atomic<uint64_t>[n_slots]);
    for (size_t k = 0; k < n_slots; k++) t->slot_tag[k].store(0, std::memory_order_relaxed);
    hipError_t e = dev_malloc((void**)&t->data, t->slot_elems() * n_slots * sizeof(u64));
    if (e != hipSuccess) {
        delete t;
        return fail(ZKW_ERR_OOM, "zkw_trace_create: hipMalloc of %zu bytes failed: %s",
                    n_cols * n_rows * n_slots * 8, hipGetErrorString(e));
    }
    ctx_retain(ctx);
    *out = t;
    return ZKW_OK;
}

extern "C" int zkw_trace_create(zkw_ctx* ctx, size_t n_rows, size_t n_slots, zkw_trace** out) {
    return zkw_trace_create_with_columns(ctx, n_rows, RC_COLS, n_slots, out);
}

extern "C" void zkw_trace_free(zkw_trace* t) {
    if (!t) return;
    (void)hipSetDevice(t->ctx->device);
    (void)hipStreamSynchronize(t->ctx->stream);
    if (t->data) dev_free(t->data);
    zkw_ctx* owner = t->ctx;
    delete t;
    ctx_release(owner);
}

extern "C" size_t zkw_trace_num_rows(const zkw_trace* t) { return t ? t->n_rows : 0; }
extern "C" size_t zkw_trace_num_cols(const zkw_trace* t) { return t ? t->n_cols : 0; }
extern "C" size_t zkw_trace_num_slots(const zkw_trace* t) { return t ? t->n_slots : 0; }
extern "C" const uint64_t* zkw_trace_device_ptr(const zkw_trace* t, size_t slot) {
    if (!t || slot >= t->n_slots) return nullptr;
    return t->slot_for_write(slot, 0);
}

extern "C" int zkw_trace_get(const zkw_trace* t, size_t slot, uint32_t first_col, uint32_t n_cols, uint64_t* dst) {
    if (!t || !dst || slot >= t->n_slots || (size_t)first_col + n_cols > t->n_cols) return fail(ZKW_ERR_INVALID, "zkw_trace_get: bad argument");
    zkw_ctx* ctx = t->ctx;
    HIP_TRY(hipSetDevice(ctx->device));
    const u64* src = t->data + slot * t->slot_elems() + (size_t)first_col * t->n_rows;
    HIP_TRY(ctx->copy_async(dst, src, (size_t)n_cols * t->n_rows * sizeof(u64), ctx->ptr_mode == ZKW_PTR_DEVICE ? hipMemcpyDeviceToDevice : hipMemcpyDeviceToHost));
    return ctx->sync_if_host();
}

extern "C" int zkw_ram_synthesize(zkw_ctx* ctx, const zkw_ram_witness* w, size_t first_instance, size_t n_instances,
                                  zkw_trace* t, size_t first_slot) {
    if (!ctx || !w || !t || w->ctx != ctx || t->ctx->device != ctx->device) return fail(ZKW_ERR_INVALID, "zkw_ram_synthesize: bad argument");
    if (first_instance + n_instances > w->n_instances) return fail(ZKW_ERR_INVALID, "instance range out of bounds");
    if (n_instances > t->n_slots) return fail(ZKW_ERR_INVALID, "more instances (%zu) than trace slots (%zu)", n_instances, t->n_slots);
    const u32 capacity = w->capacity;
    const size_t n_rows = t->n_rows;
    if (RC_MIN_ROWS(capacity) > n_rows)
        return fail(ZKW_ERR_INVALID, "capacity %u needs %llu rows, trace has %zu", capacity,
                    (unsigned long long)RC_MIN_ROWS(capacity), n_rows);
    if (n_rows & 1) return fail(ZKW_ERR_INVALID, "trace length must be even (it is a power of two in every circuit)");
    if (n_instances == 0) return ZKW_OK;
    HIP_TRY(hipSetDevice(ctx->device));
    const size_t n_blocks = w->offsets.size() - 1;
    size_t b_first = 0;
    while (b_first + 1 < n_blocks && w->inst_offsets[b_first + 1] <= first_instance) b_first++;
    size_t b_end = b_first + 1;
    while (b_end < n_blocks && w->inst_offsets[b_end] < first_instance + n_instances) b_end++;
    const size_t win = std::min(w->zcap, w->sqcap);
    if (w->offsets[b_end] - w->offsets[b_first] > win) {
        size_t b_mid = b_first + 1;
        while (b_mid + 1 < b_end && w->offsets[b_mid + 1] - w->offsets[b_first] <= win) b_mid++;
        const size_t n_head = w->inst_offsets[b_mid] - first_instance;
        ZKW_TRY(zkw_ram_synthesize(ctx, w, first_instance, n_head, t, first_slot));
        return zkw_ram_synthesize(ctx, w, first_instance + n_head, n_instances - n_head, t, first_slot + n_head);
    }
    ZKW_TRY(ram_gp_blocks(ctx, w, b_first, b_end, w->zbuf_l, w->zbuf_r));
    const size_t z_base = w->offsets[b_first];
    {
        const size_t cnt = w->offsets[b_end] - z_base;
        Prof _p(ctx, "k_gather_encode");
        ZKW_LAUNCH(ctx, k_gather_encode, blocks_for(cnt, 256), 256, w->unsorted_q, w->perm + z_base, cnt, w->sq_win, (u64*)nullptr);
    }
    ZKW_TRY(launch_check("k_gather_encode"));
    const u32 rstride = (u32)RC_REGION_STRIDE(capacity);
    const u32 n_tiles = (rstride + 255) / 256;
    u32 *d_hist = nullptr, *d_nd = nullptr;
    ZKW_TRY(ctx->scratch_t<u32>("synth_hist", n_instances * 256, &d_hist));
    ZKW_TRY(ctx->scratch_t<u32>("synth_nd", n_instances * n_tiles, &d_nd));
    HIP_TRY(ctx->memset_async(d_hist, 0, n_instances * 256 * sizeof(u32)));
    SlotClaims claims(t);
    std::vector<SynthJob> jobs(n_instances);
    size_t b = b_first;
    for (size_t k = 0; k < n_instances; k++) {
        const size_t idx = first_instance + k;
        while (b + 1 < n_blocks && w->inst_offsets[b + 1] <= idx) b++;
        const size_t lo = w->offsets[b], nb = w->offsets[b + 1] - lo;
        SynthJob& j = jobs[k];
        j.inst = w->instances + idx;
        j.sorted_q = w->sq_win + (lo - z_base);
        j.unsorted_q = w->unsorted_q + lo;
        j.unsorted_caps = w->unsorted_caps + 4 * lo;
        j.sorted_caps = w->sorted_caps + 4 * lo;
        j.u_mark = w->unsorted_marks + 12 * idx;
        j.s_mark = w->sorted_marks + 12 * idx;
        j.challenges = w->challenges + 18 * b;
        j.lhs_z = w->zbuf_l + 2 * (lo - z_base);
        j.rhs_z = w->zbuf_r + 2 * (lo - z_base);
        j.n_block = nb;
        {
            const uint64_t tag = ((uint64_t)ZKW_CIRCUIT_RAM_PERMUTATION << 56) ^ ((uint64_t)capacity << 24) ^ (uint64_t)n_rows ^ 0x5A00000000000000ull;
            const size_t slot = (first_slot + k) % t->n_slots;
            bool clean = false;
            j.trace = claims.claim(slot, tag, &clean);
            j.tail_clean = clean;
        }
        j.hist = d_hist + 256 * k;
        j.nd_tiles = d_nd + (size_t)n_tiles * k;
        j.public_input = w->public_inputs + 4 * idx;
        j.first_inst = w->instances + w->inst_offsets[b];
    }
    SynthJob* d_jobs = nullptr;
    ZKW_TRY(ctx->upload("synth_jobs", jobs, &d_jobs));
    const unsigned nj = (unsigned)n_instances;
    const dim3 g64((rstride + 63) / 64, nj), g256(n_tiles, nj);
    { Prof _p(ctx, "k_ram_nd_tiles"); ZKW_LAUNCH_D(ctx, (k_ram_nd_tiles), "k_ram_nd_tiles", g256, 256, 0, d_jobs, capacity); }
    ZKW_TRY(launch_check("k_ram_nd_tiles"));
    { Prof _p(ctx, "k_ram_nd_scan"); ZKW_LAUNCH(ctx, k_ram_nd_scan, nj, 64, d_jobs, (int)nj, n_tiles); }
    ZKW_TRY(launch_check("k_ram_nd_scan"));
    { Prof _p(ctx, "k_ram_fill_poseidon"); ZKW_LAUNCH_D(ctx, (k_ram_fill_poseidon<0>), "k_ram_fill_poseidon", g64, 64, 0, d_jobs, capacity, n_rows); }
    ZKW_TRY(launch_check("k_ram_fill_poseidon<0>"));
    { Prof _p(ctx, "k_ram_fill_poseidon"); ZKW_LAUNCH_D(ctx, (k_ram_fill_poseidon<1>), "k_ram_fill_poseidon", g64, 64, 0, d_jobs, capacity, n_rows); }
    ZKW_TRY(launch_check("k_ram_fill_poseidon<1>"));
    { Prof _p(ctx, "k_ram_fill_A"); ZKW_LAUNCH_D(ctx, (k_ram_fill_A), "k_ram_fill_A", g256, 256, 0, d_jobs, capacity, n_rows); }
    ZKW_TRY(launch_check("k_ram_fill_A"));
    { Prof _p(ctx, "k_ram_fill_B"); ZKW_LAUNCH_D(ctx, (k_ram_fill_B), "k_ram_fill_B", g256, 256, 0, d_jobs, capacity, n_rows); }
    ZKW_TRY(launch_check("k_ram_fill_B"));
    { Prof _p(ctx, "k_ram_fill_C"); ZKW_LAUNCH_D(ctx, (k_ram_fill_C), "k_ram_fill_C", g256, 256, 0, d_jobs, capacity, n_rows); }
    ZKW_TRY(launch_check("k_ram_fill_C"));
    { Prof _p(ctx, "k_ram_fill_D"); const unsigned d_tiles = (unsigned)((rstride + RC_D_TILES * 256 - 1) / (RC_D_TILES * 256));
      ZKW_LAUNCH(ctx, k_ram_fill_D, nj * (d_tiles + 1), 256, d_jobs, nj, d_tiles, capacity, n_rows); }
    ZKW_TRY(launch_check("k_ram_fill_D"));
    { Prof _p(ctx, "k_ram_fill_tail"); ZKW_LAUNCH(ctx, k_ram_fill_tail, nj * ((RC_G + RC_L + 1) * TAIL_CHUNKS), 256, d_jobs, capacity, n_rows); }
    ZKW_TRY(launch_check("k_ram_fill_tail"));
    return claims.commit_if(ctx->sync_if_host());
}


extern "C" int zkw_ram_check_satisfied(zkw_ctx* ctx, const zkw_trace* t, size_t slot, uint32_t capacity,
                                       uint64_t* n_violations, uint64_t* first_bad) {
    if (!ctx || !t || t->ctx->device != ctx->device || slot >= t->n_slots || !n_violations)
        return fail(ZKW_ERR_INVALID, "zkw_ram_check_satisfied: bad argument");
    if (RC_MIN_ROWS(capacity) > t->n_rows) return fail(ZKW_ERR_INVALID, "capacity does not fit the trace");
    return check_satisfied<SpecRam>(ctx, t, slot, capacity, n_violations, first_bad);
}

extern "C" int zkw_decommit_sorter_check_satisfied(zkw_ctx* ctx, const zkw_trace* t, size_t slot, uint32_t capacity,
                                                   uint64_t* n_violations, uint64_t* first_bad) {
    if (!ctx || !t || t->ctx->device != ctx->device || slot >= t->n_slots || !n_violations)
        return fail(ZKW_ERR_INVALID, "zkw_decommit_sorter_check_satisfied: bad argument");
    if (DS_MIN_ROWS(capacity) > t->n_rows) return fail(ZKW_ERR_INVALID, "capacity does not fit the trace");
    return check_satisfied<SpecDecommitSorter>(ctx, t, slot, capacity, n_violations, first_bad);
}

extern "C" int zkw_closed_form_public_inputs(zkw_ctx* ctx, uint8_t circuit_type, const void* instances, size_t n, uint64_t* compact,
                                             uint64_t* public_inputs) {
    if (!ctx || !compact || !public_inputs || (n && !instances)) return fail(ZKW_ERR_INVALID, "zkw_closed_form_public_inputs: null argument");
    if (n == 0) return ZKW_OK;
    HIP_TRY(hipSetDevice(ctx->device));
    switch (circuit_type) {
        case 3: return closed_form_from_records<CfDecommitter>(ctx, instances, n, compact, public_inputs);
        case 5: return closed_form_from_records<CfPrecompile<ZKW_PRECOMPILE_KECCAK256>>(ctx, instances, n, compact, public_inputs);
        case 6: return closed_form_from_records<CfPrecompile<ZKW_PRECOMPILE_SHA256>>(ctx, instances, n, compact, public_inputs);
        case 7: return closed_form_from_records<CfPrecompile<ZKW_PRECOMPILE_ECRECOVER>>(ctx, instances, n, compact, public_inputs);
        case 10: return closed_form_from_records<CfStorageApplication>(ctx, instances, n, compact, public_inputs);
        case 13: return closed_form_from_records<CfLinearHasher>(ctx, instances, n, compact, public_inputs);
        default: break;
    }
    return fail(ZKW_ERR_INVALID, "zkw_closed_form_public_inputs: circuit type %u keeps its compact forms in its witness (2, 4, 8, 9, 11, 12) "
                                 "or is not a base-layer circuit with a closed form here", (unsigned)circuit_type);
}

extern "C" int zkw_commit_encodings(zkw_ctx* ctx, const uint64_t* enc, size_t n_items, uint32_t item_len, uint64_t* out) {
    if (!ctx || !out || (n_items && item_len && !enc)) return fail(ZKW_ERR_INVALID, "zkw_commit_encodings: null argument");
    if (n_items == 0) return ZKW_OK;
    HIP_TRY(hipSetDevice(ctx->device));
    const u64* d_enc = nullptr;
    u64* d_out = nullptr;
    ZKW_TRY(ctx->in("ce_enc", enc, n_items * item_len + 1, &d_enc));
    ZKW_TRY(ctx->out("ce_out", out, n_items * 4, &d_out));
    { Prof _p(ctx, "k_commit_encodings"); ZKW_LAUNCH(ctx, k_commit_encodings, blocks_for(n_items, 64), 64, d_enc, n_items, item_len, d_out); }
    ZKW_TRY(launch_check("k_commit_encodings"));
    ZKW_TRY(ctx->finish_out(out, d_out, n_items * 4));
    return ctx->sync_if_host();
}

extern "C" int zkw_encode_recursion_requests(zkw_ctx* ctx, uint64_t circuit_type, const uint64_t* public_inputs, size_t n,
                                             uint64_t* enc) {
    if (!ctx || !enc || !public_inputs) return fail(ZKW_ERR_INVALID, "zkw_encode_recursion_requests: null argument");
    if (n == 0) return ZKW_OK;
    HIP_TRY(hipSetDevice(ctx->device));
    const u64* d_pi = nullptr;
    u64* d_enc = nullptr;
    ZKW_TRY(ctx->in("rr_pi", public_inputs, n * 4, &d_pi));
    ZKW_TRY(ctx->out("rr_enc", enc, n * 8, &d_enc));
    { Prof _p(ctx, "k_encode_recursion"); ZKW_LAUNCH(ctx, k_encode_recursion, blocks_for(n, 64), 64, circuit_type, d_pi, n, d_enc); }
    ZKW_TRY(launch_check("k_encode_recursion"));
    ZKW_TRY(ctx->finish_out(enc, d_enc, n * 8));
    return ctx->sync_if_host();
}

extern "C" int zkw_encode_callstack_entries(zkw_ctx* ctx, const zkw_callstack_entry* entries, size_t n, uint64_t* enc) {
    if (!ctx || !enc || !entries) return fail(ZKW_ERR_INVALID, "zkw_encode_callstack_entries: null argument");
    if (n == 0) return ZKW_OK;
    HIP_TRY(hipSetDevice(ctx->device));
    const zkw_callstack_entry* d_e = nullptr;
    u64* d_enc = nullptr;
    ZKW_TRY(ctx->in("cs_e", entries, n, &d_e));
    ZKW_TRY(ctx->out("cs_enc", enc, n * 32, &d_enc));
    { Prof _p(ctx, "k_encode_callstack"); hipLaunchKernelGGL(k_encode_callstack, dim3(blocks_for(n, 64)), dim3(64), 0, ctx->stream, d_e, n, d_enc); }
    ZKW_TRY(launch_check("k_encode_callstack"));
    ZKW_TRY(ctx->finish_out(enc, d_enc, n * 32));
    return ctx->sync_if_host();
}

extern "C" int zkw_callstack_simulate(zkw_ctx* ctx, const uint8_t* is_push, size_t n_ops, const zkw_callstack_entry* pushed,
                                      size_t n_pushed, uint64_t* previous_state, uint64_t* new_state, uint32_t* depth,
                                      uint64_t* round_states, uint32_t* entry_index) {
    if (!ctx || !is_push || !previous_state || !new_state || !depth || !round_states || !entry_index || (n_pushed && !pushed))
        return fail(ZKW_ERR_INVALID, "zkw_callstack_simulate: null argument");
    if (n_ops == 0) return ZKW_OK;
    if (n_ops >= (1ull << 31)) return fail(ZKW_ERR_INVALID, "too many stack operations");
    HIP_TRY(hipSetDevice(ctx->device));
    const uint8_t* d_ops = nullptr;
    const zkw_callstack_entry* d_e = nullptr;
    ZKW_TRY(ctx->in("st_ops", is_push, n_ops, &d_ops));
    if (n_pushed) ZKW_TRY(ctx->in("st_e", pushed, n_pushed, &d_e));
    u32 *d_depth = nullptr, *d_rank = nullptr, *d_meta = nullptr, *d_pd = nullptr, *d_pid = nullptr, *d_sd = nullptr, *d_sid = nullptr,
        *d_parent = nullptr, *d_node = nullptr;
    u64* d_rounds = nullptr;
    void* tmp = nullptr;
    const size_t tmp_bytes = radix_temp_bytes(n_ops);
    ZKW_TRY(ctx->scratch_t<u32>("st_depth", n_ops, &d_depth));
    ZKW_TRY(ctx->scratch_t<u32>("st_rank", n_ops, &d_rank));
    ZKW_TRY(ctx->scratch_t<u32>("st_meta", 4, &d_meta));
    ZKW_TRY(ctx->scratch_t<u32>("st_pd", n_ops, &d_pd));
    ZKW_TRY(ctx->scratch_t<u32>("st_pid", n_ops, &d_pid));
    ZKW_TRY(ctx->scratch_t<u32>("st_sd", n_ops, &d_sd));
    ZKW_TRY(ctx->scratch_t<u32>("st_sid", n_ops, &d_sid));
    ZKW_TRY(ctx->scratch_t<u32>("st_parent", n_ops, &d_parent));
    ZKW_TRY(ctx->scratch_t<u32>("st_node", n_ops, &d_node));
    ZKW_TRY(ctx->scratch_t<u64>("st_rounds", n_ops * 48, &d_rounds));
    ZKW_TRY(ctx->scratch("st_tmp", tmp_bytes + 256, &tmp));
    u64 *d_prefix = nullptr, *d_totals = nullptr;
    ZKW_TRY(ctx->scratch_t<u64>("st_prefix", 2 * (n_ops + 1), &d_prefix));
    ZKW_TRY(ctx->scratch_t<u64>("st_totals", 2, &d_totals));
    HIP_TRY(ctx->memset_async(d_meta, 0, 4 * sizeof(u32)));
    ZKW_TRY((sum_prefix<2>(ctx, "k_stack_prefix", StackDelta{d_ops}, n_ops, d_prefix, d_totals)));
    { Prof _p(ctx, "k_stack_depth"); hipLaunchKernelGGL(k_stack_depth, dim3(blocks_for(n_ops, 256)), dim3(256), 0, ctx->stream, d_ops, n_ops, d_prefix, d_depth, d_rank, d_meta); }
    ZKW_TRY(launch_check("k_stack_depth"));
    u32 meta[3];
    ZKW_TRY(ctx->read_small(meta, d_meta, sizeof meta));
    if (meta[2]) return fail(ZKW_ERR_INVALID, "pop from the empty callstack (circuit_encodings/src/lib.rs:619)");
    const u32 n_push = meta[0], max_depth = meta[1];
    if (n_push > n_pushed) return fail(ZKW_ERR_INVALID, "%u pushes but only %zu entries", n_push, n_pushed);
    const unsigned grid = blocks_for(n_ops, 256);
    if (n_push) {
        { Prof _p(ctx, "k_stack_push_keys"); hipLaunchKernelGGL(k_stack_push_keys, dim3(grid), dim3(256), 0, ctx->stream, d_ops, n_ops, d_depth, d_rank, d_pd, d_pid); }
        ZKW_TRY(launch_check("k_stack_push_keys"));
        unsigned bits = 1;
        while ((1ull << bits) <= max_depth) bits++;
        { Prof _p(ctx, "radix_sort"); ZKW_TRY(radix_sort_pairs<u32>(ctx, tmp, tmp_bytes, d_pd, d_sd, d_pid, d_sid, n_push, bits)); }
    }
    { Prof _p(ctx, "k_stack_links"); hipLaunchKernelGGL(k_stack_links, dim3(grid), dim3(256), 0, ctx->stream, d_ops, n_ops, d_depth, d_rank, d_sd, d_sid, d_meta, d_parent, d_node); }
    ZKW_TRY(launch_check("k_stack_links"));
    for (u32 d = 1; d <= max_depth; d++) {
        Prof _p(ctx, "k_stack_level");
        hipLaunchKernelGGL(k_stack_level, dim3(blocks_for(n_push, 64)), dim3(64), 0, ctx->stream, d_e, d_pd, d_parent, d_meta, d, d_rounds);
    }
    ZKW_TRY(launch_check("k_stack_level"));
    u64 *d_prev = nullptr, *d_new = nullptr, *d_rs = nullptr;
    u32 *d_dep = nullptr, *d_idx = nullptr;
    ZKW_TRY(ctx->out("st_o_prev", previous_state, n_ops * 12, &d_prev));
    ZKW_TRY(ctx->out("st_o_new", new_state, n_ops * 12, &d_new));
    ZKW_TRY(ctx->out("st_o_rs", round_states, n_ops * 48, &d_rs));
    ZKW_TRY(ctx->out("st_o_dep", depth, n_ops, &d_dep));
    ZKW_TRY(ctx->out("st_o_idx", entry_index, n_ops, &d_idx));
    { Prof _p(ctx, "k_stack_emit"); hipLaunchKernelGGL(k_stack_emit, dim3(grid), dim3(256), 0, ctx->stream, d_ops, n_ops, d_depth, d_parent, d_node, d_rounds, d_meta, d_prev, d_new, d_dep, d_rs, d_idx); }
    ZKW_TRY(launch_check("k_stack_emit"));
    ZKW_TRY(ctx->finish_out(previous_state, d_prev, n_ops * 12));
    ZKW_TRY(ctx->finish_out(new_state, d_new, n_ops * 12));
    ZKW_TRY(ctx->finish_out(round_states, d_rs, n_ops * 48));
    ZKW_TRY(ctx->finish_out(depth, d_dep, n_ops));
    ZKW_TRY(ctx->finish_out(entry_index, d_idx, n_ops));
    return ctx->sync_if_host();
}

extern "C" int zkw_vm_slice_instances(zkw_ctx* ctx, const zkw_vm_tracer_streams* in, zkw_vm_instance* instances,
                                      uint32_t* memory_read_index, uint32_t* memory_write_index, uint64_t* n_reads, uint64_t* n_writes) {
    if (!ctx || !in || !instances || !in->snapshot_cycles || in->n_snapshots < 2 || ((memory_read_index == nullptr) != (memory_write_index == nullptr)))
        return fail(ZKW_ERR_INVALID, "zkw_vm_slice_instances: bad argument");
    for (int k = 0; k < ZKW_VM_NUM_STREAMS; k++)
        if (in->stream_len[k] && !in->stream_cycles[k]) return fail(ZKW_ERR_INVALID, "zkw_vm_slice_instances: stream %d has no cycle stamps", k);
    const size_t n_mem = in->stream_len[ZKW_VMS_MEMORY];
    if (n_mem >= (1ull << 32)) return fail(ZKW_ERR_INVALID, "too many memory queries");
    if ((n_mem && (!in->vm_memory_queries || !in->memory_queue_tails)) || (in->n_decommit_states && (!in->decommit_state_cycles || !in->decommit_queue_tails)) ||
        (in->n_callstack_sponges && (!in->callstack_sponge_cycles || !in->callstack_sponge_states)) ||
        (in->n_storage_log_states && (!in->storage_log_state_cycles || !in->storage_log_states)))
        return fail(ZKW_ERR_INVALID, "zkw_vm_slice_instances: a stream's payload is missing");
    HIP_TRY(hipSetDevice(ctx->device));
    const size_t n_inst = in->n_snapshots - 1;
    VmSliceJob job;
    job.s = *in;
    ZKW_TRY(ctx->in("vm_snap", in->snapshot_cycles, in->n_snapshots, &job.s.snapshot_cycles));
    static const char* names[ZKW_VM_NUM_STREAMS] = {"vm_c0", "vm_c1", "vm_c2", "vm_c3", "vm_c4", "vm_c5", "vm_c6", "vm_c7"};
    for (int k = 0; k < ZKW_VM_NUM_STREAMS; k++) ZKW_TRY(ctx->in(names[k], in->stream_cycles[k], in->stream_len[k], &job.s.stream_cycles[k]));
    ZKW_TRY(ctx->in("vm_memq", in->vm_memory_queries, n_mem, &job.s.vm_memory_queries));
    ZKW_TRY(ctx->in("vm_memt", in->memory_queue_tails, n_mem * 12, &job.s.memory_queue_tails));
    ZKW_TRY(ctx->in("vm_decc", in->decommit_state_cycles, in->n_decommit_states, &job.s.decommit_state_cycles));
    ZKW_TRY(ctx->in("vm_dect", in->decommit_queue_tails, in->n_decommit_states * 12, &job.s.decommit_queue_tails));
    ZKW_TRY(ctx->in("vm_csc", in->callstack_sponge_cycles, in->n_callstack_sponges, &job.s.callstack_sponge_cycles));
    ZKW_TRY(ctx->in("vm_css", in->callstack_sponge_states, in->n_callstack_sponges * 12, &job.s.callstack_sponge_states));
    ZKW_TRY(ctx->in("vm_slc", in->storage_log_state_cycles, in->n_storage_log_states, &job.s.storage_log_state_cycles));
    ZKW_TRY(ctx->in("vm_sls", in->storage_log_states, in->n_storage_log_states, &job.s.storage_log_states));
    u32 *d_tiles = nullptr, *d_prefix = nullptr, *d_ri = nullptr, *d_wi = nullptr;
    u64* d_total = nullptr;
    const u32 n_tiles = (u32)((n_mem + VM_TILE) / VM_TILE);
    ZKW_TRY(ctx->scratch_t<u32>("vm_tiles", n_tiles, &d_tiles));
    ZKW_TRY(ctx->scratch_t<u32>("vm_prefix", n_mem + 1, &d_prefix));
    ZKW_TRY(ctx->scratch_t<u64>("vm_total", 1, &d_total));
    if (memory_read_index) {
        ZKW_TRY(ctx->out("vm_ri", memory_read_index, n_mem, &d_ri));
        ZKW_TRY(ctx->out("vm_wi", memory_write_index, n_mem, &d_wi));
    }
    { Prof _p(ctx, "k_vm_rw_tile_counts"); ZKW_LAUNCH(ctx, k_vm_rw_tile_counts, n_tiles, 256, job.s.vm_memory_queries, (u64)n_mem, d_tiles); }
    ZKW_TRY(launch_check("k_vm_rw_tile_counts"));
    { Prof _p(ctx, "k_vm_rw_scan_tiles"); ZKW_LAUNCH(ctx, k_vm_rw_scan_tiles, 1, 1024, d_tiles, n_tiles, d_total); }
    ZKW_TRY(launch_check("k_vm_rw_scan_tiles"));
    { Prof _p(ctx, "k_vm_rw_scatter"); ZKW_LAUNCH(ctx, k_vm_rw_scatter, n_tiles, 256, job.s.vm_memory_queries, (u64)n_mem, d_tiles, d_prefix, d_ri, d_wi); }
    ZKW_TRY(launch_check("k_vm_rw_scatter"));
    job.read_prefix = d_prefix;
    ZKW_TRY(ctx->out("vm_inst", instances, n_inst, &job.out));
    { Prof _p(ctx, "k_vm_slice"); ZKW_LAUNCH(ctx, k_vm_slice, blocks_for(n_inst, 64), 64, job); }
    ZKW_TRY(launch_check("k_vm_slice"));
    ZKW_TRY(ctx->finish_out(instances, job.out, n_inst));
    if (memory_read_index) {
        ZKW_TRY(ctx->finish_out(memory_read_index, d_ri, n_mem));
        ZKW_TRY(ctx->finish_out(memory_write_index, d_wi, n_mem));
    }
    if (n_reads || n_writes) {
        u64 total = 0;
        ZKW_TRY(ctx->read_small(&total, d_total, 8));
        if (n_reads) *n_reads = total;
        if (n_writes) *n_writes = n_mem - total;
    }
    return ctx->sync_if_host();
}
```

Measured before the change: 3082.

## Pair Poseidon2 partial rounds and use 32-bit uniform column addressing in RAM fills

Poseidon2 partial rounds are processed in pairs, reusing the 32-bit split sums and diagonal products of the first round to build the second round's state, so only one set of reductions is done per pair. This cuts multiply and reduce work in the partial-round chain used by the trace fill and the checker. Trace cell addressing is also rewritten to compute column bases as wave-uniform scalars via readfirstlane, with 32-bit row byte offsets, which lowers per-store 64-bit address arithmetic. A guard rejects traces at or above 2^29 rows, since the new addressing cannot reach them. The paired-round algebra is more intricate and depends on the shift constants (the shl_add_hi path for shifts above 4), so a mistake there would corrupt the trace silently.

New measurement: 3118 (median of 3 runs). Within noise of the previous version (+1.2%).

```diff
diff --git a/era_zkevm_test_harness_amd/csrc/poseidon2.cuh b/era_zkevm_test_harness_amd/csrc/poseidon2.cuh
--- a/era_zkevm_test_harness_amd/csrc/poseidon2.cuh
+++ b/era_zkevm_test_harness_amd/csrc/poseidon2.cuh
@@ -83,6 +83,11 @@
     asm("v_mad_u64_u32 %0, %1, %2, -1, %3" : "=v"(r), "=s"(dead) : "v"(f), "v"(r));
     return r;
 }
+__device__ __forceinline__ u64 shl_add_hi(u32 w, u32 sh, u64 acc) {
+    u32 hi;
+    asm("v_lshl_add_u32 %0, %1, %2, %3" : "=v"(hi) : "v"(w), "s"(sh), "v"((u32)(acc >> 32)));
+    return ((u64)hi << 32) | (u32)acc;
+}
 __device__ __forceinline__ void m4_plane(u32 a0, u32 a1, u32 a2, u32 a3, u64 y[4]) {
     const u64 t0 = mad_acc1(a0, (u64)a1), t1 = mad_acc1(a2, (u64)a3);
     const u64 t2 = mad_acc2(a1, t1), t3 = mad_acc2(a3, t0);
@@ -156,6 +161,50 @@
 GL_HD void partial_round(u64 s[12], int r) {
     s[0] = LAT ? gl::pow7_lat(gl::add_canon(s[0], rc_at(12 * r))) : gl::pow7(gl::add_canon(s[0], rc_at(12 * r)));
     internal(s);
+}
+
+template <class Sink>
+GL_HD void partial_rounds(u64 s[12], int r0, Sink&& sink) {
+#if defined(__HIP_DEVICE_COMPILE__) && !defined(P2_LINEAR_WIDE) && !defined(P2_PARTIAL_EAGER)
+    static_assert(P2_PARTIAL_ROUNDS % 2 == 0, "partial rounds go in pairs");
+    constexpr u32 SH[12] = P2_INTERNAL_DIAG_SHIFTS_INIT;
+    for (int k = 0; k < P2_PARTIAL_ROUNDS; k += 2) {
+        s[0] = gl::pow7(gl::add_canon(s[0], rc_at(12 * (r0 + k))));
+        sink(k, s[0]);
+        u64 sl = (u64)(u32)s[0], sh = s[0] >> 32;
+#pragma unroll
+        for (int i = 1; i < 12; i++) { sl = mad_acc1((u32)s[i], sl); sh = mad_acc1((u32)(s[i] >> 32), sh); }
+        u64 L[12], H[12];
+#pragma unroll
+        for (int i = 0; i < 12; i++) {
+            L[i] = SH[i] ? mad_acc((u32)s[i], 1u << SH[i], sl) : mad_acc1((u32)s[i], sl);
+            H[i] = SH[i] ? mad_acc((u32)(s[i] >> 32), 1u << SH[i], sh) : mad_acc1((u32)(s[i] >> 32), sh);
+        }
+        s[0] = gl::pow7(gl::add_canon(wp_reduce(L[0], H[0]), rc_at(12 * (r0 + k + 1))));
+        sink(k + 1, s[0]);
+        u64 tl = (u64)(u32)s[0], th = s[0] >> 32;
+#pragma unroll
+        for (int i = 1; i < 12; i++) { tl += L[i]; th += H[i]; }
+        s[0] = wp_reduce(mad_acc((u32)s[0], 1u << SH[0], tl), mad_acc((u32)(s[0] >> 32), 1u << SH[0], th));
+#pragma unroll
+        for (int i = 1; i < 12; i++) {
+            u64 l, h;
+            if (SH[i] <= 4) {
+                l = (L[i] << SH[i]) + tl; h = (H[i] << SH[i]) + th;
+            } else {
+                l = shl_add_hi((u32)(L[i] >> 32), SH[i], mad_acc((u32)L[i], 1u << SH[i], tl));
+                h = shl_add_hi((u32)(H[i] >> 32), SH[i], mad_acc((u32)H[i], 1u << SH[i], th));
+            }
+            s[i] = wp_reduce(l, h);
+        }
+    }
+#else
+    for (int k = 0; k < P2_PARTIAL_ROUNDS; k++) {
+        s[0] = gl::pow7(gl::add_canon(s[0], rc_at(12 * (r0 + k))));
+        sink(k, s[0]);
+        internal(s);
+    }
+#endif
 }
 
 template <bool LAT = false>
diff --git a/era_zkevm_test_harness_amd/csrc/ram_circuit_kernels.cuh b/era_zkevm_test_harness_amd/csrc/ram_circuit_kernels.cuh
--- a/era_zkevm_test_harness_amd/csrc/ram_circuit_kernels.cuh
+++ b/era_zkevm_test_harness_amd/csrc/ram_circuit_kernels.cuh
@@ -54,12 +54,40 @@
 
 #define TR(col, row) trace[(size_t)(col) * n_rows + (row)]
 
-__device__ __forceinline__ void zero_gap_row(u64* trace, size_t n_rows, size_t row) {
-    for (int col = 0; col < RC_G + RC_L; col++) TR(col, row) = 0;
-}
-__device__ __forceinline__ void zero_gap_row_n(u64* trace, size_t n_rows, size_t row, int n_cols) {
-    for (int col = 0; col < n_cols; col++) TR(col, row) = 0;
-}
+__device__ __forceinline__ u64 uni64(u64 v) {
+    return ((u64)(u32)__builtin_amdgcn_readfirstlane((int)(v >> 32)) << 32) | (u32)__builtin_amdgcn_readfirstlane((int)v);
+}
+#if defined(ZKW_RAM_FLAT_CELLS)
+struct Cells {
+    u64* trace;
+    size_t n_rows;
+    __device__ __forceinline__ Cells(u64* t, size_t n) : trace(t), n_rows(n) {}
+    __device__ __forceinline__ u64& operator()(int col, u32 row) const { return TR(col, row); }
+};
+typedef u64 u64x2 __attribute__((ext_vector_type(2)));
+typedef u64x2 cell_pair;
+#else
+typedef __attribute__((address_space(1))) u64 g_u64;
+typedef __attribute__((address_space(1))) char g_char;
+typedef u64 u64x2 __attribute__((ext_vector_type(2)));
+typedef __attribute__((address_space(1))) u64x2 cell_pair;
+struct Cells {
+    g_char* trace;
+    u32 col_bytes;
+    __device__ __forceinline__ Cells(u64* t, size_t n) : trace((g_char*)uni64((u64)t)), col_bytes((u32)n * 8u) {}
+    __device__ __forceinline__ g_u64& operator()(int col, u32 row) const {
+        g_char* base = (g_char*)uni64((u64)(trace + (u64)(u32)col * col_bytes));
+        return *(g_u64*)(base + row * 8u);
+    }
+};
+#endif
+
+__device__ __forceinline__ void zero_gap_row_n(const Cells& T, u32 row, int n_cols) {
+    for (int col = 0; col < n_cols; col++) T(col, row) = 0;
+}
+__device__ __forceinline__ void zero_gap_row(const Cells& T, u32 row) { zero_gap_row_n(T, row, RC_G + RC_L); }
+__device__ __forceinline__ void zero_gap_row(u64* trace, size_t n_rows, size_t row) { zero_gap_row_n(Cells(trace, n_rows), (u32)row, RC_G + RC_L); }
+__device__ __forceinline__ void zero_gap_row_n(u64* trace, size_t n_rows, size_t row, int n_cols) { zero_gap_row_n(Cells(trace, n_rows), (u32)row, n_cols); }
 
 __device__ __forceinline__ void hist_bytes(u32* sh_hist, u32 x) {
     atomicAdd(&sh_hist[x & 0xFF], 1u);
@@ -67,41 +95,43 @@
     atomicAdd(&sh_hist[(x >> 16) & 0xFF], 1u);
     atomicAdd(&sh_hist[x >> 24], 1u);
 }
-__device__ __forceinline__ void put_bytes(u64* trace, size_t n_rows, size_t row, int col0, u32 x) {
-    TR(col0, row) = x & 0xFF;
-    TR(col0 + 1, row) = (x >> 8) & 0xFF;
-    TR(col0 + 2, row) = (x >> 16) & 0xFF;
-    TR(col0 + 3, row) = x >> 24;
-}
+__device__ __forceinline__ void put_bytes(const Cells& T, u32 row, int col0, u32 x) {
+    T(col0, row) = x & 0xFF;
+    T(col0 + 1, row) = (x >> 8) & 0xFF;
+    T(col0 + 2, row) = (x >> 16) & 0xFF;
+    T(col0 + 3, row) = x >> 24;
+}
+__device__ __forceinline__ void put_bytes(u64* trace, size_t n_rows, size_t row, int col0, u32 x) { put_bytes(Cells(trace, n_rows), (u32)row, col0, x); }
 __device__ __forceinline__ void hist_flush(u32* sh_hist, u32* g_hist) {
     __syncthreads();
     for (int t = threadIdx.x; t < 256; t += blockDim.x)
         if (sh_hist[t]) atomicAdd(&g_hist[t], sh_hist[t]);
 }
 
-__device__ __forceinline__ void fill_flattened_poseidon(u64* trace, size_t n_rows, size_t row, u64 s[12]) {
+__device__ __forceinline__ void fill_flattened_poseidon(const Cells& T, u32 row, u64 s[12]) {
     int pos = 0;
 #pragma unroll
-    for (int k = 0; k < 12; k++) TR(pos++, row) = gl::canon(s[k]);
+    for (int k = 0; k < 12; k++) T(pos++, row) = gl::canon(s[k]);
     p2::external(s);
     int r = 0;
     for (int k = 0; k < P2_HALF_FULL_ROUNDS; k++, r++) {
         p2::full_round(s, r);
 #pragma unroll
-        for (int j = 0; j < 12; j++) TR(pos + j, row) = gl::canon(s[j]);
+        for (int j = 0; j < 12; j++) T(pos + j, row) = gl::canon(s[j]);
         pos += 12;
     }
-    for (int k = 0; k < P2_PARTIAL_ROUNDS; k++, r++) {
-        s[0] = gl::pow7(gl::add_canon(s[0], p2::rc_at(12 * r)));
-        TR(pos++, row) = gl::canon(s[0]);
-        p2::internal(s);
-    }
+    p2::partial_rounds(s, r, [&](int k, u64 x) { T(pos + k, row) = gl::canon(x); });
+    pos += P2_PARTIAL_ROUNDS;
+    r += P2_PARTIAL_ROUNDS;
     for (int k = 0; k < P2_HALF_FULL_ROUNDS; k++, r++) {
         p2::full_round(s, r);
 #pragma unroll
-        for (int j = 0; j < 12; j++) TR(pos + j, row) = gl::canon(s[j]);
+        for (int j = 0; j < 12; j++) T(pos + j, row) = gl::canon(s[j]);
         pos += 12;
     }
+}
+__device__ __forceinline__ void fill_flattened_poseidon(u64* trace, size_t n_rows, size_t row, u64 s[12]) {
+    fill_flattened_poseidon(Cells(trace, n_rows), (u32)row, s);
 }
 
 template <int SIDE>
@@ -111,13 +141,13 @@
     for (int t = threadIdx.x; t < 256; t += blockDim.x) sh_hist[t] = 0;
     __syncthreads();
     const SynthJob job = jobs[vb.y];
+    const Cells T(job.trace, n_rows);
     const u32 i = vb.x * blockDim.x + threadIdx.x;
+    const u32 row = (u32)(SIDE == 0 ? RC_ROW_PU : RC_ROW_PS) * (u32)RC_REGION_STRIDE(capacity) + i;
     if (i < capacity) {
-        u64* trace = job.trace;
         const zkw_ram_instance* in = job.inst;
         const size_t first = in->first_item, m = in->num_items;
         const bool can_pop = i < m;
-        const size_t row = (size_t)(SIDE == 0 ? RC_ROW_PU : RC_ROW_PS) * RC_REGION_STRIDE(capacity) + i;
         const zkw_mem_query* qs = SIDE == 0 ? job.unsorted_q : job.sorted_q;
         const u64* caps = SIDE == 0 ? job.unsorted_caps : job.sorted_caps;
         u64 s[12];
@@ -131,26 +161,26 @@
         const u64* prev_cap = i == 0 ? (SIDE == 0 ? ri.uh : ri.sh) + 8 : caps + 4 * (first + (i - 1 < m ? i - 1 : m - 1));
 #pragma unroll
         for (int k = 0; k < 4; k++) s[8 + k] = prev_cap[k];
-        fill_flattened_poseidon(trace, n_rows, row, s);
+        fill_flattened_poseidon(T, row, s);
         zkw_mem_query q;
         memset(&q, 0, sizeof q);
         if (can_pop) q = job.sorted_q[first + i];
         if (SIDE == 0) {
-            TR(RC_PU_idx, row) = q.index; TR(RC_PU_v0, row) = q.value[0]; TR(RC_PU_v1, row) = q.value[1];
-            put_bytes(trace, n_rows, row, RC_PU_idx_b0, q.index);
-            put_bytes(trace, n_rows, row, RC_PU_v0_b0, q.value[0]);
-            put_bytes(trace, n_rows, row, RC_PU_v1_b0, q.value[1]);
+            T(RC_PU_idx, row) = q.index; T(RC_PU_v0, row) = q.value[0]; T(RC_PU_v1, row) = q.value[1];
+            put_bytes(T, row, RC_PU_idx_b0, q.index);
+            put_bytes(T, row, RC_PU_v0_b0, q.value[0]);
+            put_bytes(T, row, RC_PU_v1_b0, q.value[1]);
             hist_bytes(sh_hist, q.index); hist_bytes(sh_hist, q.value[0]); hist_bytes(sh_hist, q.value[1]);
         } else {
-            if (!job.tail_clean) for (int c = 130; c < RC_G; c++) TR(c, row) = 0;
-            put_bytes(trace, n_rows, row, RC_PS_ts_b0, q.timestamp);
-            put_bytes(trace, n_rows, row, RC_PS_page_b0, q.page);
-            put_bytes(trace, n_rows, row, RC_PS_v4_b0, q.value[4]);
+            if (!job.tail_clean) for (int c = 130; c < RC_G; c++) T(c, row) = 0;
+            put_bytes(T, row, RC_PS_ts_b0, q.timestamp);
+            put_bytes(T, row, RC_PS_page_b0, q.page);
+            put_bytes(T, row, RC_PS_v4_b0, q.value[4]);
             hist_bytes(sh_hist, q.timestamp); hist_bytes(sh_hist, q.page); hist_bytes(sh_hist, q.value[4]);
         }
-        if (!job.tail_clean) for (int c = RC_G + 12; c < RC_G + RC_L; c++) TR(c, row) = 0;
+        if (!job.tail_clean) for (int c = RC_G + 12; c < RC_G + RC_L; c++) T(c, row) = 0;
     } else if (i < RC_REGION_STRIDE(capacity)) {
-        if (!job.tail_clean) zero_gap_row(job.trace, n_rows, (size_t)(SIDE == 0 ? RC_ROW_PU : RC_ROW_PS) * RC_REGION_STRIDE(capacity) + i);
+        if (!job.tail_clean) zero_gap_row(T, row);
     }
     hist_flush(sh_hist, job.hist);
 }
@@ -206,19 +236,20 @@
     sh_hist[threadIdx.x] = 0;
     __syncthreads();
     const SynthJob job = jobs[vb.y];
+    const Cells T(job.trace, n_rows);
     const u32 i = vb.x * blockDim.x + threadIdx.x;
+    const u32 row = (u32)RC_ROW_A * (u32)RC_REGION_STRIDE(capacity) + i;
     const u64* lhs_z_all = job.lhs_z;
     const u64* rhs_z_all = job.rhs_z;
     const size_t n_total = job.n_block;
     if (i < capacity) {
-        u64* trace = job.trace;
         const zkw_ram_instance* in = job.inst;
-        const size_t first = in->first_item, m = in->num_items, row = (size_t)RC_ROW_A * RC_REGION_STRIDE(capacity) + i;
+        const size_t first = in->first_item, m = in->num_items;
         CycleCtx c;
         cycle_ctx(job, i, c, true);
         const u64 rw = c.q.rw_flag ? 1 : 0, ptr = c.q.value_is_pointer ? 1 : 0;
 #pragma unroll
-        for (int k = 0; k < 8; k++) { TR(RC_A_eu0 + k, row) = c.eu[k]; TR(RC_A_ts + k, row) = c.es[k]; }
+        for (int k = 0; k < 8; k++) { T(RC_A_eu0 + k, row) = c.eu[k]; T(RC_A_ts + k, row) = c.es[k]; }
         for (int r = 0; r < 2; r++) {
             const u64* ch = job.challenges + 9 * r;
             u64 lc = ch[8], rc = ch[8];
@@ -232,26 +263,26 @@
             const u64 nl = gl::canon(gl::mul(pl, lc)), nr = gl::canon(gl::mul(pr, rc));
             const int o = r * (RC_A_lc1 - RC_A_lc0);
 #pragma unroll
-            for (int k = 1; k < 9; k++) TR(RC_A_G_c0_1 + (k - 1) + r * (RC_A_G_c1_1 - RC_A_G_c0_1), row) = ch[k];
-            TR(RC_A_lc0 + o, row) = gl::canon(lc); TR(RC_A_P_lhs0 + o, row) = pl; TR(RC_A_nl0 + o, row) = nl;
-            TR(RC_A_lhs0 + o, row) = c.can_pop ? nl : pl;
-            TR(RC_A_rc0 + o, row) = gl::canon(rc); TR(RC_A_P_rhs0 + o, row) = pr; TR(RC_A_nr0 + o, row) = nr;
-            TR(RC_A_rhs0 + o, row) = c.can_pop ? nr : pr;
-        }
-        TR(RC_A_rw, row) = rw; TR(RC_A_ptr, row) = ptr; TR(RC_A_idx, row) = c.q.index;
-        TR(RC_A_v2, row) = c.q.value[2]; TR(RC_A_v3, row) = c.q.value[3]; TR(RC_A_v0, row) = c.q.value[0];
-        TR(RC_A_v5_b3c, row) = c.q.value[5] >> 24; TR(RC_A_can_pop, row) = c.can_pop ? 1 : 0;
-        put_bytes(trace, n_rows, row, RC_A_v2_b0, c.q.value[2]);
-        put_bytes(trace, n_rows, row, RC_A_v3_b0, c.q.value[3]);
-        put_bytes(trace, n_rows, row, RC_A_v5_b0, c.q.value[5]);
+            for (int k = 1; k < 9; k++) T(RC_A_G_c0_1 + (k - 1) + r * (RC_A_G_c1_1 - RC_A_G_c0_1), row) = ch[k];
+            T(RC_A_lc0 + o, row) = gl::canon(lc); T(RC_A_P_lhs0 + o, row) = pl; T(RC_A_nl0 + o, row) = nl;
+            T(RC_A_lhs0 + o, row) = c.can_pop ? nl : pl;
+            T(RC_A_rc0 + o, row) = gl::canon(rc); T(RC_A_P_rhs0 + o, row) = pr; T(RC_A_nr0 + o, row) = nr;
+            T(RC_A_rhs0 + o, row) = c.can_pop ? nr : pr;
+        }
+        T(RC_A_rw, row) = rw; T(RC_A_ptr, row) = ptr; T(RC_A_idx, row) = c.q.index;
+        T(RC_A_v2, row) = c.q.value[2]; T(RC_A_v3, row) = c.q.value[3]; T(RC_A_v0, row) = c.q.value[0];
+        T(RC_A_v5_b3c, row) = c.q.value[5] >> 24; T(RC_A_can_pop, row) = c.can_pop ? 1 : 0;
+        put_bytes(T, row, RC_A_v2_b0, c.q.value[2]);
+        put_bytes(T, row, RC_A_v3_b0, c.q.value[3]);
+        put_bytes(T, row, RC_A_v5_b0, c.q.value[5]);
         hist_bytes(sh_hist, c.q.value[2]); hist_bytes(sh_hist, c.q.value[3]); hist_bytes(sh_hist, c.q.value[5]);
         constexpr int NA = ROW_SLOTS[RC_ROW_A];
         if (!job.tail_clean) {
-            for (int col = NA; col < RC_G; col++) TR(col, row) = 0;
-            for (int col = RC_G + 12; col < RC_G + RC_L; col++) TR(col, row) = 0;
+            for (int col = NA; col < RC_G; col++) T(col, row) = 0;
+            for (int col = RC_G + 12; col < RC_G + RC_L; col++) T(col, row) = 0;
         }
     } else if (i < RC_REGION_STRIDE(capacity)) {
-        if (!job.tail_clean) zero_gap_row(job.trace, n_rows, (size_t)RC_ROW_A * RC_REGION_STRIDE(capacity) + i);
+        if (!job.tail_clean) zero_gap_row(T, row);
     }
     hist_flush(sh_hist, job.hist);
 }
@@ -261,29 +292,29 @@
     sh_hist[threadIdx.x] = 0;
     __syncthreads();
     const SynthJob job = jobs[vb.y];
+    const Cells T(job.trace, n_rows);
     const u32 i = vb.x * blockDim.x + threadIdx.x;
+    const u32 row = (u32)RC_ROW_B * (u32)RC_REGION_STRIDE(capacity) + i;
     if (i < capacity) {
-        u64* trace = job.trace;
-        const size_t row = (size_t)RC_ROW_B * RC_REGION_STRIDE(capacity) + i;
         CycleCtx c;
         cycle_ctx(job, i, c, false);
-        put_bytes(trace, n_rows, row, RC_B_v6_b0, c.q.value[6]);
-        put_bytes(trace, n_rows, row, RC_B_v7_b0, c.q.value[7]);
-        TR(RC_B_es4, row) = c.es[4]; TR(RC_B_v1, row) = c.q.value[1]; TR(RC_B_v5_b3c, row) = c.q.value[5] >> 24;
-        TR(RC_B_es5, row) = c.es[5]; TR(RC_B_v2, row) = c.q.value[2];
-        TR(RC_B_es6, row) = c.es[6]; TR(RC_B_v3, row) = c.q.value[3];
+        put_bytes(T, row, RC_B_v6_b0, c.q.value[6]);
+        put_bytes(T, row, RC_B_v7_b0, c.q.value[7]);
+        T(RC_B_es4, row) = c.es[4]; T(RC_B_v1, row) = c.q.value[1]; T(RC_B_v5_b3c, row) = c.q.value[5] >> 24;
+        T(RC_B_es5, row) = c.es[5]; T(RC_B_v2, row) = c.q.value[2];
+        T(RC_B_es6, row) = c.es[6]; T(RC_B_v3, row) = c.q.value[3];
         const u32 d0 = c.q.timestamp - c.pq.timestamp;
-        TR(RC_B_d0, row) = d0; put_bytes(trace, n_rows, row, RC_B_d0_b0, d0);
-        TR(RC_B_bw0, row) = c.q.timestamp < c.pq.timestamp ? 1 : 0;
-        TR(RC_B_ts, row) = c.q.timestamp; TR(RC_B_P_ts, row) = c.pq.timestamp;
+        T(RC_B_d0, row) = d0; put_bytes(T, row, RC_B_d0_b0, d0);
+        T(RC_B_bw0, row) = c.q.timestamp < c.pq.timestamp ? 1 : 0;
+        T(RC_B_ts, row) = c.q.timestamp; T(RC_B_P_ts, row) = c.pq.timestamp;
         hist_bytes(sh_hist, c.q.value[6]); hist_bytes(sh_hist, c.q.value[7]); hist_bytes(sh_hist, d0);
         constexpr int NB = ROW_SLOTS[RC_ROW_B];
         if (!job.tail_clean) {
-            for (int col = NB; col < RC_G; col++) TR(col, row) = 0;
-            for (int col = RC_G + 12; col < RC_G + RC_L; col++) TR(col, row) = 0;
+            for (int col = NB; col < RC_G; col++) T(col, row) = 0;
+            for (int col = RC_G + 12; col < RC_G + RC_L; col++) T(col, row) = 0;
         }
     } else if (i < RC_REGION_STRIDE(capacity)) {
-        if (!job.tail_clean) zero_gap_row(job.trace, n_rows, (size_t)RC_ROW_B * RC_REGION_STRIDE(capacity) + i);
+        if (!job.tail_clean) zero_gap_row(T, row);
     }
     hist_flush(sh_hist, job.hist);
 }
@@ -331,7 +362,9 @@
     sh_hist[threadIdx.x] = 0;
     __syncthreads();
     const SynthJob job = jobs[vb.y];
+    const Cells T(job.trace, n_rows);
     const u32 i = vb.x * blockDim.x + threadIdx.x;
+    const u32 row = (u32)RC_ROW_C * (u32)RC_REGION_STRIDE(capacity) + i;
     const bool live = i < capacity;
     CycleCtx c;
     c.can_pop = false;
@@ -347,22 +380,20 @@
     u32 before = __popcll(bal & ((1ull << lane) - 1));
     for (int w = 0; w < wave; w++) before += sh_wave[w];
     if (live) {
-        u64* trace = job.trace;
         const zkw_ram_instance* in = job.inst;
-        const size_t row = (size_t)RC_ROW_C * RC_REGION_STRIDE(capacity) + i;
         const u64 rw = c.q.rw_flag ? 1 : 0, ptr = c.q.value_is_pointer ? 1 : 0;
         const u64 bw0 = c.q.timestamp < c.pq.timestamp ? 1 : 0;
         const u64 t1 = (u64)c.pq.index + bw0, bw1 = (u64)c.q.index < t1 ? 1 : 0;
         const u32 d1 = (u32)((u64)c.q.index - t1);
         const u64 t2 = (u64)c.pq.page + bw1, bw2 = (u64)c.q.page < t2 ? 1 : 0;
         const u32 d2 = (u32)((u64)c.q.page - t2);
-        TR(RC_C_d1, row) = d1; put_bytes(trace, n_rows, row, RC_C_d1_b0, d1);
-        TR(RC_C_d2, row) = d2; put_bytes(trace, n_rows, row, RC_C_d2_b0, d2);
+        T(RC_C_d1, row) = d1; put_bytes(T, row, RC_C_d1_b0, d1);
+        T(RC_C_d2, row) = d2; put_bytes(T, row, RC_C_d2_b0, d2);
         hist_bytes(sh_hist, d1); hist_bytes(sh_hist, d2);
-        TR(RC_C_bw1, row) = bw1; TR(RC_C_bw2, row) = bw2; TR(RC_C_bw0, row) = bw0;
-        TR(RC_C_idx, row) = c.q.index; TR(RC_C_P_idx, row) = c.pq.index;
-        TR(RC_C_page, row) = c.q.page; TR(RC_C_P_page, row) = c.pq.page;
-        TR(RC_C_can_pop, row) = c.can_pop ? 1 : 0;
+        T(RC_C_bw1, row) = bw1; T(RC_C_bw2, row) = bw2; T(RC_C_bw0, row) = bw0;
+        T(RC_C_idx, row) = c.q.index; T(RC_C_P_idx, row) = c.pq.index;
+        T(RC_C_page, row) = c.q.page; T(RC_C_P_page, row) = c.pq.page;
+        T(RC_C_can_pop, row) = c.can_pop ? 1 : 0;
         u64 x[14];
         x[0] = gl::canon(gl::sub(c.q.index, c.pq.index));
         x[1] = gl::canon(gl::sub(c.q.page, c.pq.page));
@@ -381,8 +412,8 @@
             inv = gl::mul(inv, x[k] ? x[k] : 1);
         }
         const u64 z_idx = x[0] == 0, z_page = x[1] == 0, same = z_idx & z_page;
-        TR(RC_C_w_idx, row) = w[0]; TR(RC_C_z_idx, row) = z_idx;
-        TR(RC_C_w_page, row) = w[1]; TR(RC_C_z_page, row) = z_page; TR(RC_C_same, row) = same;
+        T(RC_C_w_idx, row) = w[0]; T(RC_C_z_idx, row) = z_idx;
+        T(RC_C_w_page, row) = w[1]; T(RC_C_z_page, row) = z_page; T(RC_C_same, row) = same;
         const int C_VAL[5] = {RC_C_es3, RC_C_es4, RC_C_es5, RC_C_es6, RC_C_v4};
         const int C_PVAL[5] = {RC_C_P_es3, RC_C_P_es4, RC_C_P_es5, RC_C_P_es6, RC_C_P_v4};
         const int C_WEQ[5] = {RC_C_w_eq0, RC_C_w_eq1, RC_C_w_eq2, RC_C_w_eq3, RC_C_w_eq4};
@@ -393,26 +424,26 @@
 #pragma unroll
         for (int k = 0; k < 5; k++) {
             zeq[k] = x[2 + k] == 0; zz[k] = x[7 + k] == 0;
-            TR(C_VAL[k], row) = val[k]; TR(C_PVAL[k], row) = c.p_val[k];
-            TR(C_WEQ[k], row) = w[2 + k]; TR(C_ZEQ[k], row) = zeq[k];
-            TR(C_WZ[k], row) = w[7 + k]; TR(C_ZZ[k], row) = zz[k];
+            T(C_VAL[k], row) = val[k]; T(C_PVAL[k], row) = c.p_val[k];
+            T(C_WEQ[k], row) = w[2 + k]; T(C_ZEQ[k], row) = zeq[k];
+            T(C_WZ[k], row) = w[7 + k]; T(C_ZZ[k], row) = zz[k];
         }
         const u64 peq = ptr == c.p_ptr, eq_a = zeq[0] & zeq[1] & zeq[2], value_equal = eq_a & zeq[3] & zeq[4] & peq;
         const u64 zz_a = zz[0] & zz[1] & zz[2], all_zero = zz_a & zz[3] & zz[4] & (1 - ptr);
-        TR(RC_C_ptr, row) = ptr; TR(RC_C_P_ptr, row) = c.p_ptr; TR(RC_C_peq, row) = peq;
-        TR(RC_C_eq_a, row) = eq_a; TR(RC_C_value_equal, row) = value_equal;
-        TR(RC_C_zz_a, row) = zz_a; TR(RC_C_all_zero, row) = all_zero; TR(RC_C_rw, row) = rw;
-        TR(RC_C_ts, row) = c.q.timestamp; TR(RC_C_w_ts, row) = w[12]; TR(RC_C_z_ts, row) = x[12] == 0;
-        TR(RC_C_w_heap, row) = w[13]; TR(RC_C_z_heap, row) = x[13] == 0; TR(RC_C_nd, row) = nd ? 1 : 0;
+        T(RC_C_ptr, row) = ptr; T(RC_C_P_ptr, row) = c.p_ptr; T(RC_C_peq, row) = peq;
+        T(RC_C_eq_a, row) = eq_a; T(RC_C_value_equal, row) = value_equal;
+        T(RC_C_zz_a, row) = zz_a; T(RC_C_all_zero, row) = all_zero; T(RC_C_rw, row) = rw;
+        T(RC_C_ts, row) = c.q.timestamp; T(RC_C_w_ts, row) = w[12]; T(RC_C_z_ts, row) = x[12] == 0;
+        T(RC_C_w_heap, row) = w[13]; T(RC_C_z_heap, row) = x[13] == 0; T(RC_C_nd, row) = nd ? 1 : 0;
         const u64 p_cnt = (u64)in->hidden_fsm_input.num_nondeterministic_writes + job.nd_tiles[vb.x] + before;
-        TR(RC_C_P_cnt, row) = p_cnt; TR(RC_C_cnt, row) = p_cnt + (nd ? 1 : 0);
+        T(RC_C_P_cnt, row) = p_cnt; T(RC_C_cnt, row) = p_cnt + (nd ? 1 : 0);
         constexpr int NC = ROW_SLOTS[RC_ROW_C];
         if (!job.tail_clean) {
-            for (int col = NC; col < RC_G; col++) TR(col, row) = 0;
-            for (int col = RC_G + 8; col < RC_G + RC_L; col++) TR(col, row) = 0;
+            for (int col = NC; col < RC_G; col++) T(col, row) = 0;
+            for (int col = RC_G + 8; col < RC_G + RC_L; col++) T(col, row) = 0;
         }
     } else if (i < RC_REGION_STRIDE(capacity)) {
-        if (!job.tail_clean) zero_gap_row(job.trace, n_rows, (size_t)RC_ROW_C * RC_REGION_STRIDE(capacity) + i);
+        if (!job.tail_clean) zero_gap_row(T, row);
     }
     if (vb.x == 0 && threadIdx.x == 0)
         for (int l = 5; l < 8; l++) { hist_bytes(sh_hist, job.inst->hidden_fsm_input.previous_value[l]); hist_bytes(sh_hist, job.inst->hidden_fsm_output.previous_value[l]); }
@@ -429,8 +460,8 @@
     }
     const SynthJob& job = jobs[(vb.x - n_jobs) / n_tiles];
     const u32 i0 = ((vb.x - n_jobs) % n_tiles) * (RC_D_TILES * 256) + threadIdx.x;
-    const size_t rs = RC_REGION_STRIDE(capacity);
-    u64* trace = job.trace;
+    const u32 rs = (u32)RC_REGION_STRIDE(capacity);
+    const Cells T(job.trace, n_rows);
     const zkw_ram_instance* in = job.inst;
     const size_t m = in->num_items;
     const RegsIn ri = regs_in(in);
@@ -453,30 +484,29 @@
     for (int k = 0; k < RC_D_TILES; k++) {
         const u32 i = i0 + 256 * k;
         if (i >= capacity) {
-            if (i < rs && !job.tail_clean) zero_gap_row(job.trace, n_rows, (size_t)RC_ROW_D * rs + i);
+            if (i < rs && !job.tail_clean) zero_gap_row(T, RC_ROW_D * rs + i);
             continue;
         }
-        const size_t row = (size_t)RC_ROW_D * rs + i;
-        const size_t rPU = (size_t)RC_ROW_PU * rs + i, rPS = (size_t)RC_ROW_PS * rs + i;
+        const u32 row = RC_ROW_D * rs + i, rPU = RC_ROW_PU * rs + i, rPS = RC_ROW_PS * rs + i;
         const bool can_pop = i < m;
         const u64 p_len = len[k];
         const u64 w_len = w[k], z_len = p_len == 0;
-        TR(RC_D_P_len_u, row) = p_len; TR(RC_D_w_lu, row) = w_len; TR(RC_D_z_lu, row) = z_len;
-        TR(RC_D_P_len_s, row) = p_len; TR(RC_D_w_ls, row) = w_len; TR(RC_D_z_ls, row) = z_len;
-        TR(RC_D_can_pop, row) = can_pop ? 1 : 0;
-        TR(RC_D_len_u, row) = p_len - (can_pop ? 1 : 0); TR(RC_D_len_s, row) = p_len - (can_pop ? 1 : 0);
-        const size_t p = i - 1 < m ? i - 1 : m - 1, rPUp = (size_t)RC_ROW_PU * rs + p, rPSp = (size_t)RC_ROW_PS * rs + p;
+        T(RC_D_P_len_u, row) = p_len; T(RC_D_w_lu, row) = w_len; T(RC_D_z_lu, row) = z_len;
+        T(RC_D_P_len_s, row) = p_len; T(RC_D_w_ls, row) = w_len; T(RC_D_z_ls, row) = z_len;
+        T(RC_D_can_pop, row) = can_pop ? 1 : 0;
+        T(RC_D_len_u, row) = p_len - (can_pop ? 1 : 0); T(RC_D_len_s, row) = p_len - (can_pop ? 1 : 0);
+        const u32 p = (u32)(i - 1 < m ? i - 1 : m - 1), rPUp = RC_ROW_PU * rs + p, rPSp = RC_ROW_PS * rs + p;
 #pragma unroll
         for (int e = 0; e < 12; e++) {
-            const u64 uo = TR(RC_PU_uo0 + e, rPU);
-            const u64 so = TR(RC_PS_so0 + e, rPS);
-            const u64 a = i == 0 ? ri.uh[e] : TR(RC_PU_uo0 + e, rPUp), b = i == 0 ? ri.sh[e] : TR(RC_PS_so0 + e, rPSp);
+            const u64 uo = T(RC_PU_uo0 + e, rPU);
+            const u64 so = T(RC_PS_so0 + e, rPS);
+            const u64 a = i == 0 ? ri.uh[e] : T(RC_PU_uo0 + e, rPUp), b = i == 0 ? ri.sh[e] : T(RC_PS_so0 + e, rPSp);
             const int o = 3 * e;
-            TR(RC_D_uo0 + o, row) = uo; TR(RC_D_P_uh0 + o, row) = a; TR(RC_D_uh0 + o, row) = can_pop ? uo : a;
-            TR(RC_D_so0 + o, row) = so; TR(RC_D_P_sh0 + o, row) = b; TR(RC_D_sh0 + o, row) = can_pop ? so : b;
+            T(RC_D_uo0 + o, row) = uo; T(RC_D_P_uh0 + o, row) = a; T(RC_D_uh0 + o, row) = can_pop ? uo : a;
+            T(RC_D_so0 + o, row) = so; T(RC_D_P_sh0 + o, row) = b; T(RC_D_sh0 + o, row) = can_pop ? so : b;
         }
         constexpr int ND = ROW_SLOTS[RC_ROW_D];
-        if (!job.tail_clean) for (int col = ND; col < RC_G + RC_L; col++) TR(col, row) = 0;
+        if (!job.tail_clean) for (int col = ND; col < RC_G + RC_L; col++) T(col, row) = 0;
     }
 }
 
@@ -488,27 +518,25 @@
     constexpr u32 PER_JOB = (RC_G + RC_L + 1) * TAIL_CHUNKS;
     const u32 bid = vb.x % PER_JOB;
     const SynthJob& job = jobs[vb.x / PER_JOB];
-    u64* trace = job.trace;
+    const Cells T(job.trace, n_rows);
     const int col = bid / TAIL_CHUNKS, ch = bid % TAIL_CHUNKS;
     if (col < RC_G + RC_L) {
         if (job.tail_clean) return;
-        const size_t bnd = (size_t)RC_BOUNDARY_ROW(capacity) + RC_BOUNDARY_ROWS;
-        const size_t n_pairs = (n_rows - bnd) / 2;
-        const size_t per = (n_pairs + TAIL_CHUNKS - 1) / TAIL_CHUNKS, lo = ch * per, hi = lo + per < n_pairs ? lo + per : n_pairs;
-        ulonglong2* c2 = reinterpret_cast<ulonglong2*>(trace + (size_t)col * n_rows + bnd);
-        const ulonglong2 z = make_ulonglong2(0, 0);
-        for (size_t k = lo + threadIdx.x; k < hi; k += 256) c2[k] = z;
+        const u32 bnd = (u32)RC_BOUNDARY_ROW(capacity) + RC_BOUNDARY_ROWS;
+        const u32 n_pairs = ((u32)n_rows - bnd) / 2;
+        const u32 per = (n_pairs + TAIL_CHUNKS - 1) / TAIL_CHUNKS, lo = ch * per, hi = lo + per < n_pairs ? lo + per : n_pairs;
+        const u64x2 z = {0, 0};
+        for (u32 k = lo + threadIdx.x; k < hi; k += 256) *(cell_pair*)&T(col, bnd + 2 * k) = z;
         return;
     }
-    u64* m = trace + (size_t)RC_MULT_COL * n_rows;
-    const size_t per = (n_rows + TAIL_CHUNKS - 1) / TAIL_CHUNKS, lo = ch * per, hi = lo + per < n_rows ? lo + per : n_rows;
-    for (size_t r = lo + threadIdx.x; r < (job.tail_clean && hi > 256 ? (lo < 256 ? 256 : lo) : hi); r += 256) {
+    const u32 per = ((u32)n_rows + TAIL_CHUNKS - 1) / TAIL_CHUNKS, lo = ch * per, hi = lo + per < n_rows ? lo + per : (u32)n_rows;
+    for (u32 r = lo + threadIdx.x; r < (job.tail_clean && hi > 256 ? (lo < 256 ? 256 : lo) : hi); r += 256) {
         u64 v = 0;
         if (r < 256) {
             v = job.hist[r];
             if (r == 0) v += (u64)RC_L * n_rows - (u64)LOOKUPS_PER_CYCLE * capacity - RC_CF_LOOKUP_CELLS;
         }
-        m[r] = v;
+        T(RC_MULT_COL, r) = v;
     }
 }
 
@@ -722,12 +750,9 @@
             for (int j = 0; j < 12; j++) ok &= gl::canon(s[j]) == CELLV(pos + j);
             pos += 12;
         }
-        for (int k = 0; k < P2_PARTIAL_ROUNDS; k++, r++) {
-            s[0] = gl::pow7(gl::add_canon(s[0], p2::rc_at(12 * r)));
-            ok &= gl::canon(s[0]) == CELLV(pos);
-            pos++;
-            p2::internal(s);
-        }
+        p2::partial_rounds(s, r, [&](int k, u64 x) { ok &= gl::canon(x) == CELLV(pos + k); });
+        pos += P2_PARTIAL_ROUNDS;
+        r += P2_PARTIAL_ROUNDS;
         for (int k = 0; k < P2_HALF_FULL_ROUNDS; k++, r++) {
             p2::full_round(s, r);
 #pragma unroll
diff --git a/era_zkevm_test_harness_amd/csrc/zkw_api.hip b/era_zkevm_test_harness_amd/csrc/zkw_api.hip
--- a/era_zkevm_test_harness_amd/csrc/zkw_api.hip
+++ b/era_zkevm_test_harness_amd/csrc/zkw_api.hip
@@ -1482,6 +1482,7 @@
         return fail(ZKW_ERR_INVALID, "capacity %u needs %llu rows, trace has %zu", capacity,
                     (unsigned long long)RC_MIN_ROWS(capacity), n_rows);
     if (n_rows & 1) return fail(ZKW_ERR_INVALID, "trace length must be even (it is a power of two in every circuit)");
+    if (n_rows >= ((size_t)1 << 29)) return fail(ZKW_ERR_INVALID, "trace length %zu: the fills address a column with 32-bit byte offsets", n_rows);
     if (n_instances == 0) return ZKW_OK;
     HIP_TRY(hipSetDevice(ctx->device));
     const size_t n_blocks = w->offsets.size() - 1;
```
